# zzzzxxxx111/Rover-SLAM

Measured on AMD Instinct MI355X. Metric: frames/s SuperPoint+LightGlue 640x480, higher is better.
Workload: dtype f32; 1 GPU; configs[3] per GPU: 33 synthetic 640x480 u8 frames resident in HBM, SuperPoint extract (Kmax=1024, thr=0.0005) + LightGlue match of 32 consecutive pairs (9 layers, filter 0.1); 32 frames counted per GPU per step; seeded synthetic weights (centred descriptor head + calibrated LightGlue law, frames shifted by multiples of 8 px); the same resident frames every step (compute-bound path, no data-depend; frames_per_gpu=32, kmax=1024, lg_fold_wo=1, pairing=calibrated

## Files before the change

include/rover_fe.h:

```cpp
#ifndef ROVER_FE_H
#define ROVER_FE_H
#include <stddef.h>
#include <stdint.h>

#ifdef __cplusplus
extern "C" {
#endif

typedef struct rfe_ctx rfe_ctx;

typedef enum {
    RFE_OK = 0,
    RFE_ERR_INVALID = -1,
    RFE_ERR_NO_DEVICE = -2,
    RFE_ERR_HIP = -3,
    RFE_ERR_IO = -4,
    RFE_ERR_NO_WEIGHTS = -5,
    RFE_ERR_OOM = -6
} rfe_status;

#define RFE_DESC_DIM 256
#define RFE_KIND_SUPERPOINT 1
#define RFE_KIND_LIGHTGLUE 2

int rfe_init(int device, rfe_ctx** out);
void rfe_destroy(rfe_ctx* ctx);
const char* rfe_last_error(rfe_ctx* ctx);
const char* rfe_version(void);

int rfe_load_weights(rfe_ctx* ctx, const char* sp_path, const char* lg_path);
int rfe_load_onnx(rfe_ctx* ctx, const char* sp_path, const char* lg_path);
int rfe_set_weights(rfe_ctx* ctx, int kind, const float* blob, int64_t count);
int64_t rfe_weight_count(int kind);
uint64_t rfe_weights_id(rfe_ctx* ctx, int kind);

typedef struct rfe_hparams {
    int32_t sp_max_keypoints;
    float sp_detection_threshold;
    int32_t sp_nms_radius;
    int32_t sp_remove_borders;
    int32_t sp_topk_always;
    int32_t lg_layers;
    int32_t lg_heads;
    float lg_filter_threshold;
} rfe_hparams;
int rfe_get_hparams(rfe_ctx* ctx, rfe_hparams* out);
int rfe_set_hparams(rfe_ctx* ctx, const rfe_hparams* in);

#define RFE_OPT_LG_FOLD_WO 1
#define RFE_OPT_LG_FP16X2 2
#define RFE_OPT_HOST_GRAPH 3
int rfe_set_option(rfe_ctx* ctx, int option, int value);
int rfe_get_option(rfe_ctx* ctx, int option, int* value);

int rfe_set_stream(rfe_ctx* ctx, void* hip_stream);
int rfe_synchronize(rfe_ctx* ctx);
int rfe_malloc(rfe_ctx* ctx, size_t bytes, void** dev_ptr);
int rfe_free(rfe_ctx* ctx, void* dev_ptr);
int rfe_host_malloc(size_t bytes, void** host_ptr);
void rfe_host_free(void* host_ptr);
int64_t rfe_workspace_bytes(rfe_ctx* ctx);
int rfe_memcpy_h2d(rfe_ctx* ctx, void* dst_dev, const void* src_host, size_t bytes);
int rfe_memcpy_d2h(rfe_ctx* ctx, void* dst_host, const void* src_dev, size_t bytes);

int rfe_extract_u8(rfe_ctx* ctx, const uint8_t* img, int H, int W, int stride, int B, int Kmax,
                   float thr, int32_t* n, int32_t* kxy, float* score, float* desc);
int rfe_extract_u8_dev(rfe_ctx* ctx, const uint8_t* img_dev, int H, int W, int stride, int B,
                       int Kmax, float thr, int32_t* n_dev, int32_t* kxy_dev, float* score_dev,
                       float* desc_dev);

int rfe_extract_f32(rfe_ctx* ctx, const float* img, int H, int W, int stride, int B, int Kmax,
                    float thr, int32_t* n, int32_t* kxy, float* score, float* desc);
int rfe_extract_f32_dev(rfe_ctx* ctx, const float* img_dev, int H, int W, int stride, int B,
                        int Kmax, float thr, int32_t* n_dev, int32_t* kxy_dev, float* score_dev,
                        float* desc_dev);

int rfe_extract_u8_bin(rfe_ctx* ctx, const uint8_t* img, int H, int W, int stride, int B, int Kmax, float thr, int32_t* n,
                       int32_t* kxy, float* score, float* desc, uint8_t* desc_bin);
int rfe_extract_u8_bin_dev(rfe_ctx* ctx, const uint8_t* img_dev, int H, int W, int stride, int B, int Kmax, float thr,
                           int32_t* n_dev, int32_t* kxy_dev, float* score_dev, float* desc_dev, uint8_t* desc_bin_dev);

#define RFE_MAX_LEVELS 16
int rfe_pyramid_geometry(int H, int W, int nlevels, float scale_factor, int32_t* level_h, int32_t* level_w, float* level_scale);
int rfe_extract_pyramid_u8(rfe_ctx* ctx, const uint8_t* img, int H, int W, int stride, int B, int nlevels, float scale_factor,
                           const int32_t* kmax, float thr, int32_t* n, int32_t* level_n, float* kpts, int32_t* octave,
                           float* score, float* desc, uint8_t* levels);
int rfe_extract_pyramid_u8_dev(rfe_ctx* ctx, const uint8_t* img_dev, int H, int W, int stride, int B, int nlevels, float scale_factor,
                               const int32_t* kmax, float thr, int32_t* n_dev, int32_t* level_n_dev, float* kpts_dev,
                               int32_t* octave_dev, float* score_dev, float* desc_dev, uint8_t* levels_dev);

int rfe_match(rfe_ctx* ctx, const float* k0n, const float* k1n, const float* d0, const float* d1,
              const int32_t* m, const int32_t* n, int P, int Mmax, int Nmax, float filter_thr,
              int32_t* S, int32_t* pairs, float* ms);
int rfe_match_dev(rfe_ctx* ctx, const float* k0n, const float* k1n, const float* d0,
                  const float* d1, const int32_t* m, const int32_t* n, int P, int Mmax, int Nmax,
                  float filter_thr, int32_t* S, int32_t* pairs, float* ms);

int rfe_match_fused(rfe_ctx* ctx, const float* kpts0_xy, int M, const float* kpts1_xy, int N,
                    const float* desc0, const float* desc1, int rows, int cols, float filter_thr,
                    float match_thresh, int32_t* vnMatches12);

int rfe_extract_match_stream_dev(rfe_ctx* ctx, const uint8_t* img_dev, int H, int W, int stride,
                                 int B, int Kmax, float thr, float filter_thr, int32_t* n_dev,
                                 int32_t* kxy_dev, float* score_dev, float* desc_dev,
                                 int32_t* S_dev, int32_t* pairs_dev, float* ms_dev);

int rfe_stereo_match(rfe_ctx* ctx, const uint8_t* imgL, const uint8_t* imgR, int H, int W, int stride,
                     const float* kL, int N, const float* kR, int Nr, const float* dL, const float* dR,
                     float mb, float mbf, float* uRight, float* depth);
int rfe_stereo_match_dev(rfe_ctx* ctx, const uint8_t* imgL, const uint8_t* imgR, int H, int W, int stride,
                         const float* kL, int N, const float* kR, int Nr, const float* dL, const float* dR,
                         float mb, float mbf, float* uRight, float* depth);

int rfe_stereo_frame_dev(rfe_ctx* ctx, const uint8_t* imgL_dev, const uint8_t* imgR_dev, int H, int W, int stride, int Kmax,
                         float thr, float filter_thr, float mb, float mbf, int reset, int32_t* n_dev, int32_t* kxy_dev,
                         float* score_dev, float* desc_dev, float* uRight_dev, float* depth_dev, int32_t* S_dev,
                         int32_t* pairs_dev, float* ms_dev);

#define RFE_STEREO_SAD_LEVEL  0
#define RFE_STEREO_SAD_LEVEL0 1
int rfe_stereo_match_pyramid(rfe_ctx* ctx, const uint8_t* levelsL, const uint8_t* levelsR, int H, int W, int nlevels, float scale_factor,
                             const float* kL, const int32_t* octL, int N, const float* kR, const int32_t* octR, int Nr,
                             const float* dL, const float* dR, float mb, float mbf, int sad_source, float* uRight, float* depth);
int rfe_stereo_match_pyramid_dev(rfe_ctx* ctx, const uint8_t* levelsL, const uint8_t* levelsR, int H, int W, int nlevels, float scale_factor,
                                 const float* kL, const int32_t* octL, int N, const float* kR, const int32_t* octR, int Nr,
                                 const float* dL, const float* dR, float mb, float mbf, int sad_source, float* uRight, float* depth);
int rfe_stereo_frame_pyramid_dev(rfe_ctx* ctx, const uint8_t* imgL_dev, const uint8_t* imgR_dev, int H, int W, int stride,
                                 int nlevels, float scale_factor, const int32_t* kmax, float thr, float filter_thr, float mb, float mbf,
                                 int sad_source, int reset, int32_t* n_dev, int32_t* level_n_dev, float* kpts_dev, int32_t* octave_dev,
                                 float* score_dev, float* desc_dev, float* uRight_dev, float* depth_dev, int32_t* S_dev,
                                 int32_t* pairs_dev, float* ms_dev);

int rfe_l2_distance_matrix(rfe_ctx* ctx, const float* a, int M, const float* b, int N, float* out);
int rfe_binarize_descriptors(rfe_ctx* ctx, const float* desc, int rows, uint8_t* out);

int rfe_search_candidates(rfe_ctx* ctx, const float* q, int Nq, const float* f, int Nf, const int32_t* offsets,
                          const int32_t* cand, const uint8_t* skip, int32_t* best_idx, float* best_dist, float* second_dist);
int rfe_distinctive_descriptors(rfe_ctx* ctx, const float* desc, const int32_t* offsets, int Np, int32_t* best, float* median);

int rfe_l2_distance_matrix_dev(rfe_ctx* ctx, const float* a_dev, int M, const float* b_dev, int N, float* out_dev);
int rfe_binarize_descriptors_dev(rfe_ctx* ctx, const float* desc_dev, int rows, uint8_t* out_dev);
int rfe_search_candidates_dev(rfe_ctx* ctx, const float* q_dev, int Nq, const float* f_dev, int Nf, const int32_t* offsets_dev,
                              const int32_t* cand_dev, const uint8_t* skip_dev, int32_t* best_idx_dev, float* best_dist_dev,
                              float* second_dist_dev);
int rfe_distinctive_descriptors_dev(rfe_ctx* ctx, const float* desc_dev, const int32_t* offsets_dev, int Np, int total, int maxn,
                                    int32_t* best_dev, float* median_dev);

int rfe_search_by_projection_dev(rfe_ctx* ctx, const float* q_dev, const float* proj_dev, const float* radius_dev,
                                 const int32_t* pred_level_dev, const uint8_t* observed_dev, int Nq, const float* f_dev,
                                 const float* kpts_dev, const int32_t* kxy_dev, const int32_t* octave_dev, const uint8_t* skip_dev, int Nf,
                                 const int32_t* nf_dev, float min_x, float min_y, float max_x, float max_y, float th_high, int cand_cap,
                                 int32_t* assign_dev, int32_t* best_idx_dev, float* best_dist_dev, float* second_dist_dev,
                                 int32_t* stats_dev);
int rfe_search_by_projection(rfe_ctx* ctx, const float* q, const float* proj, const float* radius, const int32_t* pred_level,
                             const uint8_t* observed, int Nq, const float* f, const float* kpts, const int32_t* kxy, const int32_t* octave,
                             const uint8_t* skip, int Nf, float min_x, float min_y, float max_x, float max_y, float th_high,
                             int32_t* assign, int32_t* best_idx, float* best_dist, float* second_dist, int32_t* stats);

#define RFE_PROJ_INVZ 0
#define RFE_PROJ_DIV 1
#define RFE_DIST_FLOAT 0
#define RFE_DIST_TRUNC 1
typedef struct rfe_sim3_params {
    float quat[4];
    float t[3];
    float ow[3];
    float fx, fy, cx, cy;
    float min_x, min_y, max_x, max_y;
    int32_t th;
    int32_t nlevels;
    float log_scale_factor;
    float scale_factors[RFE_MAX_LEVELS];
    int32_t proj_mode, dist_mode;
} rfe_sim3_params;
int rfe_search_by_projection_sim3_dev(rfe_ctx* ctx, const rfe_sim3_params* params, const float* q_dev, const float* pw_dev,
                                      const float* normal_dev, const float* min_dist_dev, const float* max_dist_dev,
                                      const float* scale_dist_dev, const uint8_t* valid_dev, int Np, const float* f_dev, const float* kpts_dev, const int32_t* kxy_dev,
                                      const uint8_t* matched_in_dev, int Nf, const int32_t* nf_dev, float th_accept, int cand_cap,
                                      int32_t* matched_dev, int32_t* best_idx_dev, float* best_dist_dev, float* second_dist_dev,
                                      float* proj_dev, float* radius_dev, int32_t* level_dev, int32_t* reject_dev, int32_t* stats_dev);
int rfe_search_by_projection_sim3(rfe_ctx* ctx, const rfe_sim3_params* params, const float* q, const float* pw, const float* normal,
                                  const float* min_dist, const float* max_dist, const float* scale_dist, const uint8_t* valid, int Np,
                                  const float* f,
                                  const float* kpts, const int32_t* kxy, const uint8_t* matched_in, int Nf, float th_accept,
                                  int32_t* matched, int32_t* best_idx, float* best_dist, float* second_dist, float* proj, float* radius,
                                  int32_t* level, int32_t* reject, int32_t* stats);

typedef struct rfe_pool rfe_pool;
#define RFE_POOL_AUTO 0
#define RFE_POOL_RCCL 1
#define RFE_POOL_COPY 2
int rfe_pool_create(const int* devices, int n, rfe_pool** out);
void rfe_pool_destroy(rfe_pool* pool);
const char* rfe_pool_last_error(rfe_pool* pool);
int rfe_pool_size(rfe_pool* pool);
rfe_ctx* rfe_pool_ctx(rfe_pool* pool, int member);
int rfe_pool_has_rccl(rfe_pool* pool);
int rfe_pool_set_weights(rfe_pool* pool, int kind, const float* blob, int64_t count);
int rfe_pool_load_weights(rfe_pool* pool, const char* sp_path, const char* lg_path);
int rfe_pool_set_option(rfe_pool* pool, int option, int value);
int rfe_pool_set_hparams(rfe_pool* pool, const rfe_hparams* in);
int rfe_pool_shard(int F, int n, int member, int* first_frame, int* frames, int* pairs);
int rfe_pool_extract_match_stream(rfe_pool* pool, const uint8_t* img_host, int H, int W, int stride, int F, int Kmax, float thr,
                                  float filter_thr, int transport, int32_t* n, int32_t* kxy, float* score, float* desc,
                                  int32_t* S, int32_t* pairs, float* ms);

int rfe_profile_enable(rfe_ctx* ctx, int on);
int rfe_profile_filter(rfe_ctx* ctx, const char* stage);
int rfe_profile_reset(rfe_ctx* ctx);
int rfe_profile_read(rfe_ctx* ctx, char* names, size_t names_cap, double* ms, int64_t* calls, int cap);

int rfe_k_conv3x3(rfe_ctx* ctx, const float* in_dev, int B, int H, int W, int Cin,
                  const float* w_oihw_host, const float* bias_host, int Cout, int relu, int pool,
                  float* out_dev);
int rfe_k_linear(rfe_ctx* ctx, const float* a_dev, int M, int K, const float* w_nk_host,
                 const float* bias_host, int N, int relu, float* out_dev);
int rfe_k_scoremap(rfe_ctx* ctx, const uint8_t* img_dev, int H, int W, int stride, int B,
                   float* scoremap_dev ,
                   float* nms_dev , float* descmap_dev );
int rfe_k_select(rfe_ctx* ctx, const float* nms_dev , int B, int H, int W, int Kmax, float thr, int topk_always,
                 int32_t* n_dev, int32_t* kxy_dev, float* score_dev);
int rfe_k_select_keys(rfe_ctx* ctx, const float* nms_dev , int B, int H, int W, int Kmax, float thr, int topk_always,
                      int32_t* n_dev, int32_t* kxy_dev, float* score_dev);
int rfe_k_lightglue_taps(rfe_ctx* ctx, const float* k0n, const float* k1n, const float* d0,
                         const float* d1, int M, int N, float* x0_dev, float* x1_dev,
                         float* scores_dev );

int rfe_k_lightglue_ffn(rfe_ctx* ctx, int layer, int cross, const float* x_dev, const float* second_dev, int rows, float* out_dev);
int rfe_k_attention(rfe_ctx* ctx, const float* q_dev, const float* k_dev, const float* v_dev, int ld, float* out_dev, int nseq, int Lq, int Lk,
                    const int32_t* qlen_dev, const int32_t* klen_dev, const int32_t* kv_map_dev, const float* rope_dev);
int rfe_k_lightglue_self_attention(rfe_ctx* ctx, int layer, const float* x_dev, const float* csn_dev, const int32_t* lens_dev, int nseq, int L,
                                   float* qkv_out_dev, float* ctx_out_dev, int32_t* qk_rotated);
int rfe_k_lightglue_assign(rfe_ctx* ctx, const float* sim_dev, const float* x_dev, const float* wm_dev, const float* bm_dev, const int32_t* lens_dev,
                           int P, int L, float thr, int cap, int scores_pair, int32_t sentinel, float* z_dev, float* rowlse_dev, float* collse_dev,
                           float* mx0_dev, int32_t* a0_dev, int32_t* a1_dev, int32_t* S_dev, int32_t* pairs_dev, float* ms_dev, float* scores_dev);
int rfe_k_set_lightglue_tap(rfe_ctx* ctx, int pair, float* x0_dev, float* x1_dev, float* scores_dev);
int rfe_k_pool_inject_gather_failure(rfe_pool* pool, int member);
int rfe_k_onnx_convert(const char* path, int kind, int weights_only, float* blob, rfe_hparams* hp, char* err, int errlen);

#ifdef __cplusplus
}
#endif
#endif
```

rover-slam_amd/capi.py:

```python
import ctypes as C
import os

import numpy as np

_HERE = os.path.dirname(os.path.abspath(__file__))
LIB_PATH = os.environ.get("RFE_LIBRARY") or os.path.join(_HERE, "librover_fe.so")

KIND_SUPERPOINT, KIND_LIGHTGLUE = 1, 2
OPT_LG_FOLD_WO = 1
OPT_LG_FP16X2 = 2
OPT_HOST_GRAPH = 3

EXPORTS = [
    "rfe_init", "rfe_destroy", "rfe_last_error", "rfe_version", "rfe_load_weights", "rfe_load_onnx", "rfe_set_weights",
    "rfe_weight_count", "rfe_weights_id", "rfe_get_hparams", "rfe_set_hparams", "rfe_set_option", "rfe_get_option", "rfe_set_stream", "rfe_synchronize", "rfe_malloc", "rfe_free", "rfe_host_malloc", "rfe_host_free", "rfe_workspace_bytes", "rfe_memcpy_h2d",
    "rfe_memcpy_d2h", "rfe_extract_u8", "rfe_extract_u8_dev", "rfe_extract_f32", "rfe_extract_f32_dev", "rfe_extract_u8_bin", "rfe_extract_u8_bin_dev",
    "rfe_pyramid_geometry", "rfe_extract_pyramid_u8", "rfe_extract_pyramid_u8_dev", "rfe_match", "rfe_match_dev", "rfe_match_fused",
    "rfe_extract_match_stream_dev", "rfe_stereo_match", "rfe_stereo_match_dev", "rfe_stereo_frame_dev", "rfe_stereo_match_pyramid", "rfe_stereo_match_pyramid_dev", "rfe_stereo_frame_pyramid_dev",
    "rfe_l2_distance_matrix", "rfe_binarize_descriptors",
    "rfe_search_candidates", "rfe_distinctive_descriptors",
    "rfe_l2_distance_matrix_dev", "rfe_binarize_descriptors_dev", "rfe_search_candidates_dev", "rfe_distinctive_descriptors_dev",
    "rfe_search_by_projection", "rfe_search_by_projection_dev", "rfe_search_by_projection_sim3", "rfe_search_by_projection_sim3_dev",
    "rfe_pool_create", "rfe_pool_destroy", "rfe_pool_last_error", "rfe_pool_size", "rfe_pool_ctx", "rfe_pool_has_rccl", "rfe_pool_set_weights",
    "rfe_pool_load_weights", "rfe_pool_set_option", "rfe_pool_set_hparams", "rfe_pool_shard", "rfe_pool_extract_match_stream",
    "rfe_profile_enable", "rfe_profile_filter", "rfe_profile_reset", "rfe_profile_read",
    "rfe_k_conv3x3", "rfe_k_linear", "rfe_k_scoremap", "rfe_k_select", "rfe_k_select_keys", "rfe_k_lightglue_taps", "rfe_k_set_lightglue_tap", "rfe_k_lightglue_ffn", "rfe_k_attention", "rfe_k_lightglue_self_attention", "rfe_k_lightglue_assign", "rfe_k_pool_inject_gather_failure", "rfe_k_onnx_convert",
]

if not os.path.exists(LIB_PATH):
    raise ImportError(f"{LIB_PATH} is missing: build it with `python -c 'import __graft_entry__ as g; g.build()'` "
                      "(rover-slam_amd/csrc/Makefile). There is no CPU fallback.")

lib = C.CDLL(LIB_PATH)

_vp, _fp, _ip, _u8p = C.c_void_p, C.c_void_p, C.c_void_p, C.c_void_p
lib.rfe_init.argtypes = [C.c_int, C.POINTER(C.c_void_p)]
lib.rfe_destroy.argtypes = [C.c_void_p]
lib.rfe_destroy.restype = None
lib.rfe_last_error.argtypes = [C.c_void_p]
lib.rfe_last_error.restype = C.c_char_p
lib.rfe_version.restype = C.c_char_p
lib.rfe_load_weights.argtypes = [C.c_void_p, C.c_char_p, C.c_char_p]
lib.rfe_set_weights.argtypes = [C.c_void_p, C.c_int, _fp, C.c_int64]
lib.rfe_weight_count.argtypes = [C.c_int]
lib.rfe_weight_count.restype = C.c_int64
lib.rfe_weights_id.restype = C.c_uint64
lib.rfe_weights_id.argtypes = [C.c_void_p, C.c_int]


class HParams(C.Structure):
    _fields_ = [("sp_max_keypoints", C.c_int32), ("sp_detection_threshold", C.c_float), ("sp_nms_radius", C.c_int32),
                ("sp_remove_borders", C.c_int32), ("sp_topk_always", C.c_int32), ("lg_layers", C.c_int32), ("lg_heads", C.c_int32), ("lg_filter_threshold", C.c_float)]

    def as_dict(self):
        return {k: getattr(self, k) for k, _ in self._fields_}


lib.rfe_get_hparams.argtypes = [C.c_void_p, C.POINTER(HParams)]
lib.rfe_set_hparams.argtypes = [C.c_void_p, C.POINTER(HParams)]
lib.rfe_pool_set_hparams.argtypes = [C.c_void_p, C.POINTER(HParams)]
lib.rfe_set_option.argtypes = [C.c_void_p, C.c_int, C.c_int]
lib.rfe_get_option.argtypes = [C.c_void_p, C.c_int, C.POINTER(C.c_int)]
lib.rfe_set_stream.argtypes = [C.c_void_p, C.c_void_p]
lib.rfe_synchronize.argtypes = [C.c_void_p]
lib.rfe_malloc.argtypes = [C.c_void_p, C.c_size_t, C.POINTER(C.c_void_p)]
lib.rfe_free.argtypes = [C.c_void_p, C.c_void_p]
lib.rfe_memcpy_h2d.argtypes = [C.c_void_p, C.c_void_p, C.c_void_p, C.c_size_t]
lib.rfe_memcpy_d2h.argtypes = [C.c_void_p, C.c_void_p, C.c_void_p, C.c_size_t]
_ext = [C.c_void_p, _u8p, C.c_int, C.c_int, C.c_int, C.c_int, C.c_int, C.c_float, _ip, _ip, _fp, _fp]
lib.rfe_extract_u8.argtypes = _ext
lib.rfe_extract_f32.argtypes = _ext
lib.rfe_extract_f32_dev.argtypes = _ext
lib.rfe_extract_u8_dev.argtypes = _ext
lib.rfe_extract_u8_bin.argtypes = _ext + [_u8p]
lib.rfe_extract_u8_bin_dev.argtypes = _ext + [_u8p]
lib.rfe_pyramid_geometry.argtypes = [C.c_int, C.c_int, C.c_int, C.c_float, _ip, _ip, _fp]
_pyr = [C.c_void_p, _u8p, C.c_int, C.c_int, C.c_int, C.c_int, C.c_int, C.c_float, _ip, C.c_float, _ip, _ip, _fp, _ip, _fp, _fp, _u8p]
lib.rfe_extract_pyramid_u8.argtypes = _pyr
lib.rfe_extract_pyramid_u8_dev.argtypes = _pyr
_mt = [C.c_void_p, _fp, _fp, _fp, _fp, _ip, _ip, C.c_int, C.c_int, C.c_int, C.c_float, _ip, _ip, _fp]
lib.rfe_match.argtypes = _mt
lib.rfe_match_dev.argtypes = _mt
lib.rfe_match_fused.argtypes = [C.c_void_p, _fp, C.c_int, _fp, C.c_int, _fp, _fp, C.c_int, C.c_int, C.c_float,
                                C.c_float, _ip]
lib.rfe_extract_match_stream_dev.argtypes = [C.c_void_p, _u8p, C.c_int, C.c_int, C.c_int, C.c_int, C.c_int, C.c_float,
                                             C.c_float, _ip, _ip, _fp, _fp, _ip, _ip, _fp]
_st = [C.c_void_p, _u8p, _u8p, C.c_int, C.c_int, C.c_int, _fp, C.c_int, _fp, C.c_int, _fp, _fp, C.c_float, C.c_float, _fp, _fp]
lib.rfe_stereo_match.argtypes = _st
lib.rfe_stereo_match_dev.argtypes = _st
lib.rfe_stereo_frame_dev.argtypes = [C.c_void_p, _u8p, _u8p, C.c_int, C.c_int, C.c_int, C.c_int, C.c_float, C.c_float, C.c_float, C.c_float,
                                     C.c_int, _ip, _ip, _fp, _fp, _fp, _fp, _ip, _ip, _fp]
_stp = [C.c_void_p, _u8p, _u8p, C.c_int, C.c_int, C.c_int, C.c_float, _fp, _ip, C.c_int, _fp, _ip, C.c_int, _fp, _fp, C.c_float, C.c_float,
        C.c_int, _fp, _fp]
lib.rfe_stereo_match_pyramid.argtypes = _stp
lib.rfe_stereo_match_pyramid_dev.argtypes = _stp
lib.rfe_stereo_frame_pyramid_dev.argtypes = [C.c_void_p, _u8p, _u8p, C.c_int, C.c_int, C.c_int, C.c_int, C.c_float, _ip, C.c_float, C.c_float,
                                             C.c_float, C.c_float, C.c_int, C.c_int, _ip, _ip, _fp, _ip, _fp, _fp, _fp, _fp, _ip, _ip, _fp]
lib.rfe_l2_distance_matrix.argtypes = [C.c_void_p, _fp, C.c_int, _fp, C.c_int, _fp]
lib.rfe_binarize_descriptors.argtypes = [C.c_void_p, _fp, C.c_int, _u8p]
lib.rfe_search_candidates.argtypes = [C.c_void_p, _fp, C.c_int, _fp, C.c_int, _ip, _ip, _u8p, _ip, _fp, _fp]
lib.rfe_distinctive_descriptors.argtypes = [C.c_void_p, _fp, _ip, C.c_int, _ip, _fp]
lib.rfe_l2_distance_matrix_dev.argtypes = [C.c_void_p, _fp, C.c_int, _fp, C.c_int, _fp]
lib.rfe_binarize_descriptors_dev.argtypes = [C.c_void_p, _fp, C.c_int, _u8p]
lib.rfe_search_candidates_dev.argtypes = [C.c_void_p, _fp, C.c_int, _fp, C.c_int, _ip, _ip, _u8p, _ip, _fp, _fp]
lib.rfe_distinctive_descriptors_dev.argtypes = [C.c_void_p, _fp, _ip, C.c_int, C.c_int, C.c_int, _ip, _fp]
_psq = [C.c_void_p, _fp, _fp, _fp, _ip, _u8p, C.c_int, _fp, _fp, _ip, _ip, _u8p, C.c_int]
_psb = [C.c_float, C.c_float, C.c_float, C.c_float, C.c_float]
lib.rfe_search_by_projection.argtypes = _psq + _psb + [_ip, _ip, _fp, _fp, _ip]
lib.rfe_search_by_projection_dev.argtypes = _psq + [_ip] + _psb + [C.c_int, _ip, _ip, _fp, _fp, _ip]


MAX_LEVELS = 16
PROJ_INVZ, PROJ_DIV = 0, 1
DIST_FLOAT, DIST_TRUNC = 0, 1


class Sim3Params(C.Structure):
    _fields_ = [("quat", C.c_float * 4), ("t", C.c_float * 3), ("ow", C.c_float * 3), ("fx", C.c_float), ("fy", C.c_float), ("cx", C.c_float),
                ("cy", C.c_float), ("min_x", C.c_float), ("min_y", C.c_float), ("max_x", C.c_float), ("max_y", C.c_float), ("th", C.c_int32),
                ("nlevels", C.c_int32), ("log_scale_factor", C.c_float), ("scale_factors", C.c_float * MAX_LEVELS),
                ("proj_mode", C.c_int32), ("dist_mode", C.c_int32)]


def sim3_params(quat, t, ow, intrinsics, bounds, th, scale_factors=(1.0,), log_scale_factor=0.0, proj_mode=PROJ_INVZ, dist_mode=DIST_FLOAT,
                nlevels=None):
    p = Sim3Params()
    p.quat[:] = [float(v) for v in quat]; p.t[:] = [float(v) for v in t]; p.ow[:] = [float(v) for v in ow]
    p.fx, p.fy, p.cx, p.cy = (float(v) for v in intrinsics)
    p.min_x, p.min_y, p.max_x, p.max_y = (float(v) for v in bounds)
    p.th, p.nlevels, p.log_scale_factor = int(th), len(scale_factors) if nlevels is None else int(nlevels), float(log_scale_factor)
    for l, v in enumerate(list(scale_factors)[:MAX_LEVELS]):
        p.scale_factors[l] = float(v)
    p.proj_mode, p.dist_mode = int(proj_mode), int(dist_mode)
    return p


_s3q = [C.c_void_p, C.POINTER(Sim3Params), _fp, _fp, _fp, _fp, _fp, _fp, _u8p, C.c_int, _fp, _fp, _ip, _u8p, C.c_int]
_s3o = [_ip, _ip, _fp, _fp, _fp, _fp, _ip, _ip, _ip]
lib.rfe_search_by_projection_sim3.argtypes = _s3q + [C.c_float] + _s3o
lib.rfe_search_by_projection_sim3_dev.argtypes = _s3q + [_ip, C.c_float, C.c_int] + _s3o
lib.rfe_profile_enable.argtypes = [C.c_void_p, C.c_int]
lib.rfe_profile_filter.argtypes = [C.c_void_p, C.c_char_p]
lib.rfe_profile_reset.argtypes = [C.c_void_p]
lib.rfe_profile_read.argtypes = [C.c_void_p, C.c_char_p, C.c_size_t, C.POINTER(C.c_double), C.POINTER(C.c_int64), C.c_int]
lib.rfe_k_conv3x3.argtypes = [C.c_void_p, _fp, C.c_int, C.c_int, C.c_int, C.c_int, _fp, _fp, C.c_int, C.c_int, C.c_int, _fp]
lib.rfe_k_linear.argtypes = [C.c_void_p, _fp, C.c_int, C.c_int, _fp, _fp, C.c_int, C.c_int, _fp]
lib.rfe_k_scoremap.argtypes = [C.c_void_p, _u8p, C.c_int, C.c_int, C.c_int, C.c_int, _fp, _fp, _fp]
lib.rfe_k_select.argtypes = [C.c_void_p, _fp, C.c_int, C.c_int, C.c_int, C.c_int, C.c_float, C.c_int, _ip, _ip, _fp]
lib.rfe_k_select_keys.argtypes = lib.rfe_k_select.argtypes
lib.rfe_k_lightglue_taps.argtypes = [C.c_void_p, _fp, _fp, _fp, _fp, C.c_int, C.c_int, _fp, _fp, _fp]
lib.rfe_k_set_lightglue_tap.argtypes = [C.c_void_p, C.c_int, _fp, _fp, _fp]
lib.rfe_k_lightglue_ffn.argtypes = [C.c_void_p, C.c_int, C.c_int, _fp, _fp, C.c_int, _fp]
lib.rfe_k_lightglue_self_attention.argtypes = [C.c_void_p, C.c_int, _fp, _fp, C.c_void_p, C.c_int, C.c_int, _fp, _fp, C.POINTER(C.c_int32)]
lib.rfe_k_lightglue_assign.argtypes = [C.c_void_p, _fp, _fp, _fp, _fp, _ip, C.c_int, C.c_int, C.c_float, C.c_int, C.c_int, C.c_int32,
                                       _fp, _fp, _fp, _fp, _ip, _ip, _ip, _ip, _fp, _fp]
lib.rfe_k_attention.argtypes = [C.c_void_p, _fp, _fp, _fp, C.c_int, _fp, C.c_int, C.c_int, C.c_int, C.c_void_p, C.c_void_p, C.c_void_p, _fp]


POOL_AUTO, POOL_RCCL, POOL_COPY = 0, 1, 2
lib.rfe_pool_create.argtypes = [C.POINTER(C.c_int), C.c_int, C.POINTER(C.c_void_p)]
lib.rfe_pool_destroy.argtypes = [C.c_void_p]
lib.rfe_pool_destroy.restype = None
lib.rfe_pool_last_error.argtypes = [C.c_void_p]
lib.rfe_pool_last_error.restype = C.c_char_p
lib.rfe_pool_size.argtypes = [C.c_void_p]
lib.rfe_pool_ctx.argtypes = [C.c_void_p, C.c_int]
lib.rfe_pool_ctx.restype = C.c_void_p
lib.rfe_pool_has_rccl.argtypes = [C.c_void_p]
lib.rfe_k_pool_inject_gather_failure.argtypes = [C.c_void_p, C.c_int]
lib.rfe_load_onnx.argtypes = [C.c_void_p, C.c_char_p, C.c_char_p]
lib.rfe_k_onnx_convert.argtypes = [C.c_char_p, C.c_int, C.c_int, C.POINTER(C.c_float), C.c_void_p, C.c_char_p, C.c_int]
lib.rfe_host_malloc.argtypes = [C.c_size_t, C.POINTER(C.c_void_p)]
lib.rfe_host_free.argtypes = [C.c_void_p]
lib.rfe_host_free.restype = None
lib.rfe_workspace_bytes.argtypes = [C.c_void_p]
lib.rfe_workspace_bytes.restype = C.c_int64
lib.rfe_pool_set_weights.argtypes = [C.c_void_p, C.c_int, _fp, C.c_int64]
lib.rfe_pool_load_weights.argtypes = [C.c_void_p, C.c_char_p, C.c_char_p]
lib.rfe_pool_set_option.argtypes = [C.c_void_p, C.c_int, C.c_int]
lib.rfe_pool_shard.argtypes = [C.c_int, C.c_int, C.c_int, C.POINTER(C.c_int), C.POINTER(C.c_int), C.POINTER(C.c_int)]
lib.rfe_pool_extract_match_stream.argtypes = [C.c_void_p, _u8p, C.c_int, C.c_int, C.c_int, C.c_int, C.c_int, C.c_float, C.c_float, C.c_int,
                                              _ip, _ip, _fp, _fp, _ip, _ip, _fp]


class RfeError(RuntimeError):
    pass


def _addr(a):
    if a is None:
        return None
    if isinstance(a, int):
        return a
    if isinstance(a, np.ndarray):
        assert a.flags["C_CONTIGUOUS"]
        return a.ctypes.data
    if hasattr(a, "data_ptr"):
        return a.data_ptr()
    raise TypeError(type(a))


class DevBuf:

    def __init__(self, ctx, nbytes):
        self.ctx, self.nbytes = ctx, int(nbytes)
        p = C.c_void_p()
        ctx._chk(lib.rfe_malloc(ctx.h, self.nbytes, C.byref(p)))
        self.ptr = p.value

    def upload(self, arr):
        arr = np.ascontiguousarray(arr)
        assert arr.nbytes <= self.nbytes
        self.ctx._chk(lib.rfe_memcpy_h2d(self.ctx.h, self.ptr, arr.ctypes.data, arr.nbytes))
        return self

    def download(self, shape, dtype):
        out = np.empty(shape, dtype)
        assert out.nbytes <= self.nbytes
        self.ctx._chk(lib.rfe_memcpy_d2h(self.ctx.h, out.ctypes.data, self.ptr, out.nbytes))
        return out

    def free(self):
        if self.ptr:
            lib.rfe_free(self.ctx.h, self.ptr)
            self.ptr = None


def split_levels(flat, level_h, level_w):
    out, off = [], 0
    for h, w in zip(level_h, level_w):
        out.append(flat[:, off:off + int(h) * int(w)].reshape(flat.shape[0], int(h), int(w)))
        off += int(h) * int(w)
    return out


class StereoStream:

    def __init__(self, ctx, H, W, kmax=1024, mb=0.11, mbf=0.11 * 435.0, thr=0.0005, filter_thr=0.1):
        self.ctx, self.H, self.W, self.K = ctx, H, W, kmax
        self.mb, self.mbf, self.thr, self.filter_thr = mb, mbf, thr, filter_thr
        K = kmax
        self._spec = [("n", np.int32, (2,)), ("kxy", np.int32, (2, K, 2)), ("score", np.float32, (2, K)), ("desc", np.float32, (2, K, 256)),
                      ("u_right", np.float32, (K,)), ("depth", np.float32, (K,)), ("S", np.int32, (1,)), ("pairs", np.int32, (K, 2)),
                      ("ms", np.float32, (K,))]
        self.bufs = {name: ctx.alloc(int(np.prod(shape)) * np.dtype(dt).itemsize) for name, dt, shape in self._spec}
        self.first = True

    def push(self, img_l_dev, img_r_dev, stride=None, reset=False):
        b = self.bufs
        self.ctx._chk(lib.rfe_stereo_frame_dev(self.ctx.h, _addr(img_l_dev), _addr(img_r_dev), self.H, self.W, stride or self.W, self.K,
                                               self.thr, self.filter_thr, self.mb, self.mbf, int(reset or self.first), b["n"].ptr,
                                               b["kxy"].ptr, b["score"].ptr, b["desc"].ptr, b["u_right"].ptr, b["depth"].ptr,
                                               b["S"].ptr, b["pairs"].ptr, b["ms"].ptr))
        self.first = False

    def results(self):
        self.ctx.synchronize()
        out = {name: self.bufs[name].download(shape, dt) for name, dt, shape in self._spec}
        out["S"] = int(out["S"][0])
        return out

    def close(self):
        for b in self.bufs.values():
            b.free()
        self.bufs = {}


STEREO_SAD_LEVEL, STEREO_SAD_LEVEL0 = 0, 1


class StereoPyramidStream:

    def __init__(self, ctx, H, W, nlevels=8, scale_factor=1.2, kmax=128, mb=0.11, mbf=0.11 * 435.0, thr=0.0005, filter_thr=0.1,
                 sad_source=STEREO_SAD_LEVEL):
        self.ctx, self.H, self.W, self.L, self.sf = ctx, H, W, int(nlevels), scale_factor
        self.kmax = np.full((max(self.L, 1),), int(kmax), np.int32) if np.isscalar(kmax) else np.ascontiguousarray(kmax, np.int32)
        self.mb, self.mbf, self.thr, self.filter_thr, self.sad_source = mb, mbf, thr, filter_thr, sad_source
        K = self.K = int(self.kmax.sum())
        self._spec = [("n", np.int32, (2,)), ("level_n", np.int32, (2, max(self.L, 1))), ("kpts", np.float32, (2, K, 2)),
                      ("octave", np.int32, (2, K)), ("score", np.float32, (2, K)), ("desc", np.float32, (2, K, 256)),
                      ("u_right", np.float32, (K,)), ("depth", np.float32, (K,)), ("S", np.int32, (1,)), ("pairs", np.int32, (K, 2)),
                      ("ms", np.float32, (K,))]
        self.bufs = {name: ctx.alloc(max(int(np.prod(shape)), 1) * np.dtype(dt).itemsize) for name, dt, shape in self._spec}
        self.first = True

    def push(self, img_l_dev, img_r_dev, stride=None, reset=False):
        b = self.bufs
        self.ctx._chk(lib.rfe_stereo_frame_pyramid_dev(self.ctx.h, _addr(img_l_dev), _addr(img_r_dev), self.H, self.W, stride or self.W, self.L,
                                                       self.sf, self.kmax.ctypes.data, self.thr, self.filter_thr, self.mb, self.mbf,
                                                       self.sad_source, int(reset or self.first), b["n"].ptr, b["level_n"].ptr, b["kpts"].ptr,
                                                       b["octave"].ptr, b["score"].ptr, b["desc"].ptr, b["u_right"].ptr, b["depth"].ptr,
                                                       b["S"].ptr, b["pairs"].ptr, b["ms"].ptr))
        self.first = False

    def results(self):
        self.ctx.synchronize()
        out = {name: self.bufs[name].download(shape, dt) for name, dt, shape in self._spec}
        out["S"] = int(out["S"][0])
        return out

    def close(self):
        for b in self.bufs.values():
            b.free()
        self.bufs = {}


MAX_LEVELS = 16


def pyramid_geometry(H, W, nlevels, scale_factor):
    L = max(int(nlevels), 1)
    h, w, s = np.zeros((L,), np.int32), np.zeros((L,), np.int32), np.zeros((L,), np.float32)
    rc = lib.rfe_pyramid_geometry(H, W, nlevels, scale_factor, h.ctypes.data, w.ctypes.data, s.ctypes.data)
    if rc < 0:
        raise RfeError(f"rfe_pyramid_geometry({H}, {W}, {nlevels}, {scale_factor}) failed ({rc})")
    return h, w, s


def pool_shard(F, n, member):
    a, b, c = C.c_int(), C.c_int(), C.c_int()
    rc = lib.rfe_pool_shard(F, n, member, C.byref(a), C.byref(b), C.byref(c))
    if rc < 0:
        raise RfeError(f"rfe_pool_shard({F}, {n}, {member}) failed ({rc})")
    return a.value, b.value, c.value


class Pool:

    def __init__(self, devices):
        devs = (C.c_int * len(devices))(*devices)
        h = C.c_void_p()
        rc = lib.rfe_pool_create(devs, len(devices), C.byref(h))
        if rc != 0:
            raise RfeError(f"rfe_pool_create failed ({rc}): {lib.rfe_pool_last_error(None).decode()}")
        self.h = h

    def close(self):
        if self.h:
            lib.rfe_pool_destroy(self.h)
            self.h = None

    def __del__(self):
        try:
            self.close()
        except Exception:
            pass

    def _chk(self, rc):
        if rc < 0:
            raise RfeError(f"librover_fe pool error {rc}: {lib.rfe_pool_last_error(self.h).decode()}")
        return rc

    @property
    def size(self):
        return lib.rfe_pool_size(self.h)

    @property
    def has_rccl(self):
        return bool(lib.rfe_pool_has_rccl(self.h))

    def set_weights(self, kind, blob):
        blob = np.ascontiguousarray(blob, np.float32)
        self._chk(lib.rfe_pool_set_weights(self.h, kind, blob.ctypes.data, blob.size))

    def set_option(self, option, value):
        self._chk(lib.rfe_pool_set_option(self.h, option, int(value)))

    def set_hparams(self, **kw):
        h = HParams()
        rc = lib.rfe_get_hparams(lib.rfe_pool_ctx(self.h, 0), C.byref(h))
        if rc < 0:
            raise RfeError(f"rfe_get_hparams on pool member 0 failed ({rc})")
        for k, v in kw.items():
            if not hasattr(h, k):
                raise KeyError(k)
            setattr(h, k, v)
        self._chk(lib.rfe_pool_set_hparams(self.h, C.byref(h)))

    def extract_match_stream(self, frames_u8, kmax=1024, thr=0.0005, filter_thr=0.1, transport=POOL_AUTO, with_desc=True):
        img = np.ascontiguousarray(frames_u8, np.uint8)
        F, H, W = img.shape
        P = max(F - 1, 1)
        out = {"n": np.zeros((F,), np.int32), "kxy": np.zeros((F, kmax, 2), np.int32), "S": np.zeros((P,), np.int32),
               "pairs": np.zeros((P, kmax, 2), np.int32), "ms": np.zeros((P, kmax), np.float32)}
        if with_desc:
            out["score"] = np.zeros((F, kmax), np.float32)
            out["desc"] = np.zeros((F, kmax, 256), np.float32)
        self._chk(lib.rfe_pool_extract_match_stream(self.h, img.ctypes.data, H, W, W, F, kmax, thr, filter_thr, transport, out["n"].ctypes.data,
                                                    out["kxy"].ctypes.data, out["score"].ctypes.data if with_desc else None,
                                                    out["desc"].ctypes.data if with_desc else None, out["S"].ctypes.data,
                                                    out["pairs"].ctypes.data, out["ms"].ctypes.data))
        return out


class Context:

    def __init__(self, device=0):
        h = C.c_void_p()
        rc = lib.rfe_init(device, C.byref(h))
        if rc != 0:
            raise RfeError(f"rfe_init failed ({rc}): {lib.rfe_last_error(None).decode()}")
        self.h = h

    def close(self):
        if self.h:
            lib.rfe_destroy(self.h)
            self.h = None

    def __del__(self):
        try:
            self.close()
        except Exception:
            pass

    def _chk(self, rc):
        if rc < 0:
            raise RfeError(f"librover_fe error {rc}: {lib.rfe_last_error(self.h).decode()}")
        return rc

    def set_weights(self, kind, blob):
        blob = np.ascontiguousarray(blob, np.float32)
        self._chk(lib.rfe_set_weights(self.h, kind, blob.ctypes.data, blob.size))

    def load_weights(self, sp_path=None, lg_path=None):
        self._chk(lib.rfe_load_weights(self.h, sp_path.encode() if sp_path else None, lg_path.encode() if lg_path else None))

    def get_hparams(self):
        h = HParams()
        self._chk(lib.rfe_get_hparams(self.h, C.byref(h)))
        return h.as_dict()

    def set_hparams(self, **kw):
        h = HParams()
        self._chk(lib.rfe_get_hparams(self.h, C.byref(h)))
        for k, v in kw.items():
            if not hasattr(h, k):
                raise KeyError(k)
            setattr(h, k, v)
        self._chk(lib.rfe_set_hparams(self.h, C.byref(h)))

    def set_option(self, option, value):
        self._chk(lib.rfe_set_option(self.h, option, int(value)))

    def get_option(self, option):
        v = C.c_int()
        self._chk(lib.rfe_get_option(self.h, option, C.byref(v)))
        return v.value

    def set_stream(self, stream_ptr):
        self._chk(lib.rfe_set_stream(self.h, stream_ptr))
# ... 220 lines not shown
```

rover-slam_amd/csrc/api_extract.hip:

```cpp
#include <string.h>
#include "api_internal.h"

using namespace rfe;

namespace rfe {

static void sp_layout(Bump& a, int B, int H, int W, SpBuffers& b) {
    const size_t hw = (size_t)B * H * W, cells = hw / 64;
    b.p1 = a.take<float>(hw / 4 * 64); b.a2 = a.take<float>(hw / 4 * 64);
    b.p2 = a.take<float>(hw / 16 * 64); b.a3 = a.take<float>(hw / 16 * 128);
    b.p3 = a.take<float>(cells * 128); b.a4 = a.take<float>(cells * 128); b.f4 = a.take<float>(cells * 128);
    b.pa = a.take<float>(cells * 256); b.da = a.take<float>(cells * 256); b.dmap = a.take<float>(cells * 256);
    b.logits = a.take<float>(cells * 65);
    b.smap = a.take<float>(hw); b.nmap = a.take<float>(hw); b.ss = a.take<float>(hw);
    b.mask = a.take<uint8_t>(hw); b.supp = a.take<uint8_t>(hw);
    b.cand_score = a.take<float>(hw); b.cand_idx = a.take<int32_t>(hw);
    b.sel_keys = a.take<unsigned long long>((size_t)B * 4096); b.sel_n = a.take<int32_t>(B);
}
size_t sp_ws_bytes(int B, int H, int W) { SpBuffers b; return layout_bytes([&](Bump& a) { sp_layout(a, B, H, W, b); }); }
int sp_carve(rfe_ctx* c, int B, int H, int W, SpBuffers& b) {
    return ws_carve(c, &c->ws_sp, &c->ws_sp_bytes, [&](Bump& a) { sp_layout(a, B, H, W, b); });
}

GemmArgs gemm_plain(const float* A, int lda, const float* Bw, int ldb, const float* bias, float* C, int ldc, int M, int N, int K) {
    GemmArgs g;
    memset(&g, 0, sizeof(g));
    g.A = A; g.lda = lda; g.B = Bw; g.ldb = ldb; g.bias = bias; g.C = C; g.ldc = ldc;
    g.M = M; g.N = N; g.K = K; g.alpha = 1.0f; g.batch = 1;
    return g;
}

int sp_check(rfe_ctx* c, int H, int W, int B, int Kmax) {
    if (!c) return RFE_ERR_INVALID;
    if (!c->has_sp) return fail(c, RFE_ERR_NO_WEIGHTS, "SuperPoint weights not loaded (rfe_load_weights / rfe_set_weights)");
    if (H < 8 || W < 8 || B <= 0) return fail(c, RFE_ERR_INVALID, "extract: H and W must be at least 8, B > 0");
    if (Kmax <= 0 || Kmax > 4096) return fail(c, RFE_ERR_INVALID, "extract: Kmax must be in 1..4096");
    return RFE_OK;
}

int sp_forward_maps(rfe_ctx* c, const void* img, int H, int W, int stride, int B, SpBuffers& b, bool join, bool& forked, bool img_f32, long long frame_step,
                    float thr, bool want_maps) {
    forked = false;
    int rc = sp_carve(c, B, H, W, b);
    if (rc) return rc;
    hipStream_t s = c->stream;
    const SpWeightsDev& w = c->sp;
    const int H1 = H / 2, W1 = W / 2, H2 = H1 / 2, W2 = W1 / 2, Hc = H2 / 2, Wc = W2 / 2, cells = B * Hc * Wc;
    { ProfScope p(c, "conv1ab");
      launch_conv1ab_fused(s, img, img_f32, stride, B, H, W, w.conv1a_w, w.bias[L_1A], w.packed[L_1B], w.bias[L_1B], b.p1, frame_step); }
    { ProfScope p(c, "conv2a"); launch_conv3x3(s, b.p1, B, H1, W1, 64, w.packed[L_2A], w.bias[L_2A], 64, true, kSpLayers[L_2A].pool, b.a2, L_2A); }
    { ProfScope p(c, "conv2b"); launch_conv3x3(s, b.a2, B, H1, W1, 64, w.packed[L_2B], w.bias[L_2B], 64, true, kSpLayers[L_2B].pool, b.p2, L_2B); }
    { ProfScope p(c, "conv3a"); launch_conv3x3(s, b.p2, B, H2, W2, 64, w.packed[L_3A], w.bias[L_3A], 128, true, kSpLayers[L_3A].pool, b.a3, L_3A); }
    { ProfScope p(c, "conv3b"); launch_conv3x3(s, b.a3, B, H2, W2, 128, w.packed[L_3B], w.bias[L_3B], 128, true, kSpLayers[L_3B].pool, b.p3, L_3B); }
    { ProfScope p(c, "conv4a"); launch_conv3x3(s, b.p3, B, Hc, Wc, 128, w.packed[L_4A], w.bias[L_4A], 128, true, kSpLayers[L_4A].pool, b.a4, L_4A); }
    { ProfScope p(c, "conv4b"); launch_conv3x3(s, b.a4, B, Hc, Wc, 128, w.packed[L_4B], w.bias[L_4B], 128, true, kSpLayers[L_4B].pool, b.f4, L_4B); }
    const bool fork = !(c->prof && c->prof_filter.empty());
    hipStream_t sd = fork ? c->side_stream : s;
    if (fork) { RFE_HIP(c, hipEventRecord(c->ev_fork, s)); RFE_HIP(c, hipStreamWaitEvent(sd, c->ev_fork, 0)); }
    { ProfScope p(c, "convDa", sd); launch_conv3x3(sd, b.f4, B, Hc, Wc, 128, w.packed[L_DA], w.bias[L_DA], 256, true, kSpLayers[L_DA].pool, b.da, L_DA); }
    { ProfScope p(c, "convDb", sd); launch_gemm_nt(sd, gemm_plain(b.da, 256, w.packed[L_DB], 256, w.bias[L_DB], b.dmap, 256, cells, 256, 256)); }
    { ProfScope p(c, "sp_post", sd); launch_descmap_norm(sd, b.dmap, cells); }
    if (fork) RFE_HIP(c, hipEventRecord(c->ev_join, sd));
    { ProfScope p(c, "convPa"); launch_conv3x3(s, b.f4, B, Hc, Wc, 128, w.packed[L_PA], w.bias[L_PA], 256, true, kSpLayers[L_PA].pool, b.pa, L_PA); }
    { ProfScope p(c, "convPb"); launch_gemm_nt(s, gemm_plain(b.pa, 256, w.packed[L_PB], 256, w.bias[L_PB], b.logits, 65, cells, 65, 256)); }
    { ProfScope p(c, "sp_post");
      if (B <= 4 && c->hp.sp_nms_radius == 4) {
          if (!c->sp_cnt) { RFE_HIP(c, hipMalloc((void**)&c->sp_cnt, 8 * sizeof(int32_t))); c->sp_cnt_dirty = true; }
          if (c->sp_cnt_dirty) { RFE_HIP(c, hipMemsetAsync(c->sp_cnt, 0, 8 * sizeof(int32_t), s)); c->sp_cnt_dirty = false; }
          b.tail_fused = launch_sp_tail_lat(s, b.logits, B, Hc, Wc, c->hp.sp_nms_radius, c->hp.sp_remove_borders, thr, (unsigned long long*)b.cand_score, c->sp_cnt,
                                            want_maps ? b.smap : nullptr, want_maps ? b.nmap : nullptr);
          if (b.tail_fused) c->sp_cnt_dirty = true;
      }
      if (!b.tail_fused) {
          launch_softmax65_d2s(s, b.logits, 65, B, Hc, Wc, b.smap);
          launch_nms(s, b.smap, B, 8 * Hc, 8 * Wc, c->hp.sp_nms_radius, c->hp.sp_remove_borders, b.ss, b.mask, b.supp, b.nmap);
      } }
    if (fork && join) RFE_HIP(c, hipStreamWaitEvent(s, c->ev_join, 0));
    forked = fork && !join;
    RFE_HIP(c, hipGetLastError());
    return RFE_OK;
}

int sp_forward(rfe_ctx* c, const void* img, int H, int W, int stride, int B, int Kmax, float thr,
               int32_t* n, int32_t* kxy, float* score, float* desc, uint8_t* desc_bin, bool img_f32, long long frame_step) {
    SpBuffers b;
    bool forked;
    int rc = sp_forward_maps(c, img, H, W, stride, B, b, false, forked, img_f32, frame_step, thr);
    if (rc) return rc;
    const int Hc = H / 2 / 2 / 2, Wc = W / 2 / 2 / 2, Hs = 8 * Hc, Ws = 8 * Wc;
    { ProfScope p(c, "sp_select");
      if (b.tail_fused) {
          launch_select_keys(c->stream, (const unsigned long long*)b.cand_score, c->sp_cnt, B, Hs, Ws, Kmax, c->hp.sp_topk_always != 0, n, kxy, score);
          c->sp_cnt_dirty = false;
      } else
      launch_select(c->stream, b.nmap, B, Hs, Ws, Kmax, thr, b.cand_score, b.cand_idx, n, kxy, score, (int32_t*)b.ss , c->hp.sp_topk_always != 0, b.sel_keys, b.sel_n);
      if (forked) RFE_HIP(c, hipStreamWaitEvent(c->stream, c->ev_join, 0));
      launch_desc_sample(c->stream, b.dmap, B, Hc, Wc, Hs, Ws, n, kxy, Kmax, desc, desc_bin); }
    RFE_HIP(c, hipGetLastError());
    return RFE_OK;
}

}

static int extract_check(rfe_ctx* c, const void* img, int H, int W, int stride, int B, int Kmax, const void* n, const void* kxy, const void* score,
                         const void* desc) {
    int rc = sp_check(c, H, W, B, Kmax);
    if (rc) return rc;
    if (!img || !n || !kxy || !score || !desc || stride < W) return fail(c, RFE_ERR_INVALID, "extract: null pointer or stride < W");
    RFE_HIP(c, hipSetDevice(c->device));
    return RFE_OK;
}

extern "C" int rfe_extract_u8_bin_dev(rfe_ctx* c, const uint8_t* img, int H, int W, int stride, int B, int Kmax,
                                      float thr, int32_t* n, int32_t* kxy, float* score, float* desc, uint8_t* desc_bin) {
    int rc = extract_check(c, img, H, W, stride, B, Kmax, n, kxy, score, desc);
    if (rc) return rc;
    return sp_forward(c, img, H, W, stride, B, Kmax, thr, n, kxy, score, desc, desc_bin);
}

extern "C" int rfe_extract_u8_dev(rfe_ctx* c, const uint8_t* img, int H, int W, int stride, int B, int Kmax,
                                  float thr, int32_t* n, int32_t* kxy, float* score, float* desc) {
    return rfe_extract_u8_bin_dev(c, img, H, W, stride, B, Kmax, thr, n, kxy, score, desc, nullptr);
}

extern "C" int rfe_extract_f32_dev(rfe_ctx* c, const float* img, int H, int W, int stride, int B, int Kmax,
                                   float thr, int32_t* n, int32_t* kxy, float* score, float* desc) {
    int rc = extract_check(c, img, H, W, stride, B, Kmax, n, kxy, score, desc);
    if (rc) return rc;
    return sp_forward(c, img, H, W, stride, B, Kmax, thr, n, kxy, score, desc, nullptr, true);
}

static int extract_host(rfe_ctx* c, const void* img, size_t px, int H, int W, int stride, int B, int Kmax, float thr, int32_t* n, int32_t* kxy,
                        float* score, float* desc, uint8_t* desc_bin) {
    int rc = extract_check(c, img, H, W, stride, B, Kmax, n, kxy, score, desc);
    if (rc) return rc;
    const size_t K = (size_t)B * Kmax;
    uint8_t *d_img, *d_b; int32_t *d_n, *d_k; float *d_s, *d_d;
    HostIo io(c, HostIo::PINNED);
    io.image(d_img, (const uint8_t*)img, (size_t)W * px, (size_t)B * H, (size_t)stride * px);
    io.out(d_n, n, B); io.out(d_k, kxy, K * 2); io.out(d_s, score, K);
    io.out(d_d, desc, K * 256, true);
    io.out_opt(d_b, desc_bin, K * 256);
    if ((rc = io.upload())) return rc;
    if ((rc = ensure_ws(c, &c->ws_sp, &c->ws_sp_bytes, sp_ws_bytes(B, H, W)))) return rc;
    int thr_bits; memcpy(&thr_bits, &thr, 4);
    const std::string key = px == 1 ? host_graph_key(c, "xu8", {H, W, B, Kmax, thr_bits, desc_bin != nullptr}) : host_graph_key(c, "xf32", {H, W, B, Kmax, thr_bits});
    if ((rc = run_host_graph(c, c->g_extract, key, [&] { return sp_forward(c, d_img, H, W, W, B, Kmax, thr, d_n, d_k, d_s, d_d, d_b, px == 4); }))) return rc;
    return io.download();
}

extern "C" int rfe_extract_u8(rfe_ctx* c, const uint8_t* img, int H, int W, int stride, int B, int Kmax, float thr,
                              int32_t* n, int32_t* kxy, float* score, float* desc) {
    return extract_host(c, img, 1, H, W, stride, B, Kmax, thr, n, kxy, score, desc, nullptr);
}
extern "C" int rfe_extract_u8_bin(rfe_ctx* c, const uint8_t* img, int H, int W, int stride, int B, int Kmax, float thr,
                                  int32_t* n, int32_t* kxy, float* score, float* desc, uint8_t* desc_bin) {
    return extract_host(c, img, 1, H, W, stride, B, Kmax, thr, n, kxy, score, desc, desc_bin);
}
extern "C" int rfe_extract_f32(rfe_ctx* c, const float* img, int H, int W, int stride, int B, int Kmax, float thr,
                               int32_t* n, int32_t* kxy, float* score, float* desc) {
    return extract_host(c, img, 4, H, W, stride, B, Kmax, thr, n, kxy, score, desc, nullptr);
}

extern "C" int rfe_pyramid_geometry(int H, int W, int nlevels, float scale_factor, int32_t* level_h, int32_t* level_w, float* level_scale) {
    return pyramid_geometry(H, W, nlevels, scale_factor, level_h, level_w, level_scale);
}

namespace rfe {

int pyr_check(rfe_ctx* c, int H, int W, int stride, int B, int L, float sf, const int32_t* kmax, PyrPlan& P) {
    if (!c) return RFE_ERR_INVALID;
    if (!c->has_sp) return fail(c, RFE_ERR_NO_WEIGHTS, "SuperPoint weights not loaded (rfe_load_weights / rfe_set_weights)");
    if (L < 1 || L > RFE_MAX_LEVELS) return fail(c, RFE_ERR_INVALID, "extract_pyramid: nlevels must be in 1..16");
    if (L > 1 && !(sf > 1.0f && sf <= 4.0f)) return fail(c, RFE_ERR_INVALID, "extract_pyramid: scale_factor must be in (1, 4] when nlevels > 1");
    if (H < 8 || W < 8 || B < 1 || stride < W) return fail(c, RFE_ERR_INVALID, "extract_pyramid: H and W must be at least 8, B > 0, stride >= W");
    if (!kmax) return fail(c, RFE_ERR_INVALID, "extract_pyramid: null pointer");
    P.L = L; P.Ktot = 0;
    for (int l = 0; l < L; ++l) {
        if (kmax[l] < 0 || kmax[l] > 4096) return fail(c, RFE_ERR_INVALID, "extract_pyramid: every kmax[l] must be in 0..4096");
        P.kmax[l] = kmax[l]; P.Ktot += kmax[l];
    }
    if (P.Ktot == 0) return fail(c, RFE_ERR_INVALID, "extract_pyramid: every kmax[l] is 0");
    if (pyramid_geometry(H, W, L, sf, P.h, P.w, P.s) != RFE_OK) return fail(c, RFE_ERR_INVALID, "extract_pyramid: a level rounds to zero pixels");
    P.frame = 0;
    for (int l = 0; l < L; ++l) {
        P.off[l] = P.frame; P.frame += (size_t)P.h[l] * P.w[l];
        P.run[l] = P.kmax[l] > 0 && P.h[l] >= 8 && P.w[l] >= 8;
    }
    return RFE_OK;
}

struct PyrStage { uint8_t* levels; int32_t *n[RFE_MAX_LEVELS], *kxy[RFE_MAX_LEVELS]; float *sc[RFE_MAX_LEVELS], *desc[RFE_MAX_LEVELS]; };
static void pyr_layout(Bump& a, const PyrPlan& P, int B, bool own_levels, PyrStage& st) {
    st.levels = own_levels ? a.take<uint8_t>((size_t)B * P.frame) : nullptr;
    for (int l = 0; l < P.L; ++l) {
        if (!P.run[l]) continue;
        st.n[l] = a.take<int32_t>((size_t)B); st.kxy[l] = a.take<int32_t>((size_t)B * P.kmax[l] * 2);
        st.sc[l] = a.take<float>((size_t)B * P.kmax[l]); st.desc[l] = a.take<float>((size_t)B * P.kmax[l] * 256);
    }
}

int pyr_prepare(rfe_ctx* c, int H, int W, int B, float sf, const PyrPlan& P, bool own_levels) {
    int rc;
    if ((rc = ensure_ws(c, &c->ws_sp, &c->ws_sp_bytes, sp_ws_bytes(B, H, W)))) return rc;
    PyrStage st;
    if ((rc = ensure_ws(c, &c->ws_pyr, &c->ws_pyr_bytes, layout_bytes([&](Bump& a) { pyr_layout(a, P, B, own_levels, st); })))) return rc;
    if (!c->sp_cnt) { RFE_HIP(c, hipMalloc((void**)&c->sp_cnt, 8 * sizeof(int32_t))); c->sp_cnt_dirty = true; }
    int sf_bits; memcpy(&sf_bits, &sf, 4);
    const std::string key = std::to_string(H) + "x" + std::to_string(W) + "|" + std::to_string(P.L) + "|" + std::to_string(P.L > 1 ? sf_bits : 0);
    if (P.L > 1 && key != c->ptab_key) {
        std::vector<int2> tab;
        pyramid_tables(P.L, P.h, P.w, tab, c->ptab_off);
        c->ptab_key.clear();
        const void* before = c->ws_ptab;
        if ((rc = ensure_ws(c, &c->ws_ptab, &c->ws_ptab_bytes, tab.size() * sizeof(int2)))) return rc;
        if (before == c->ws_ptab) RFE_HIP(c, hipStreamSynchronize(c->stream));
        RFE_HIP(c, hipMemcpy(c->ws_ptab, tab.data(), tab.size() * sizeof(int2), hipMemcpyHostToDevice));
        c->ptab_key = key;
    }
    return RFE_OK;
}

int pyr_forward(rfe_ctx* c, const uint8_t* img, int H, int W, int stride, int B, const PyrPlan& P, float thr, uint8_t* lv, bool copy_level0,
                int32_t* n, int32_t* level_n, float* kpts, int32_t* octave, float* score, float* desc, long long img_frame) {
    if (img_frame == 0) img_frame = (long long)stride * H;
    hipStream_t s = c->stream;
    const bool side = !(c->prof && c->prof_filter.empty());
    hipStream_t sc = side ? c->side_stream : s;
    if (side) { RFE_HIP(c, hipEventRecord(c->ev_fork, s)); RFE_HIP(c, hipStreamWaitEvent(sc, c->ev_fork, 0)); }
    { ProfScope p(c, "sp_pyramid", sc);
      if (copy_level0) launch_pyr_resample(sc, img, img_frame, stride, H, W, lv, (long long)P.frame, H, W, B, nullptr, nullptr);
      const int2* tab = (const int2*)c->ws_ptab;
      for (int l = 1; l < P.L; ++l) {
          const uint8_t* src = l == 1 ? img : lv + P.off[l - 1];
          const long long src_frame = l == 1 ? img_frame : (long long)P.frame;
          const int src_stride = l == 1 ? stride : P.w[l - 1];
          launch_pyr_resample(sc, src, src_frame, src_stride, P.h[l - 1], P.w[l - 1], lv + P.off[l], (long long)P.frame, P.h[l], P.w[l], B,
                              tab + c->ptab_off[l], tab + c->ptab_off[l] + P.w[l]);
      } }
    if (side) RFE_HIP(c, hipEventRecord(c->ev_pyr, sc));
    PyrMergeArgs m;
    memset(&m, 0, sizeof(m));
    m.L = P.L; m.Ktot = P.Ktot;
    PyrStage st;
    Bump a(c->ws_pyr);
    pyr_layout(a, P, B, lv == (uint8_t*)c->ws_pyr, st);
    int rc;
    bool joined = !side;
    for (int l = 0; l < P.L; ++l) {
        m.kmax[l] = P.kmax[l]; m.scale[l] = P.s[l];
        if (!P.run[l]) continue;
        int32_t* ln = st.n[l]; int32_t* lk = st.kxy[l]; float* ls = st.sc[l]; float* ld = st.desc[l];
        if (l >= 1 && !joined) { RFE_HIP(c, hipStreamWaitEvent(s, c->ev_pyr, 0)); joined = true; }
        if (l == 0) rc = sp_forward(c, img, H, W, stride, B, P.kmax[0], thr, ln, lk, ls, ld, nullptr, false, img_frame);
        else rc = sp_forward(c, lv + P.off[l], P.h[l], P.w[l], P.w[l], B, P.kmax[l], thr, ln, lk, ls, ld, nullptr, false, (long long)P.frame);
        if (rc) return rc;
        m.n[l] = ln; m.kxy[l] = lk; m.sc[l] = ls; m.desc_l[l] = ld;
    }
    if (!joined) RFE_HIP(c, hipStreamWaitEvent(s, c->ev_pyr, 0));
    m.n_out = n; m.level_n = level_n; m.kpts = kpts; m.octave = octave; m.score = score; m.desc = desc;
    { ProfScope p(c, "sp_merge"); launch_pyr_merge(s, m, B); }
    RFE_HIP(c, hipGetLastError());
    return RFE_OK;
}

}

static int pyr_entry_check(rfe_ctx* c, const void* img, int H, int W, int stride, int B, int nlevels, float scale_factor, const int32_t* kmax, const void* n,
                           const void* kpts, const void* octave, const void* score, const void* desc, PyrPlan& P) {
    int rc = pyr_check(c, H, W, stride, B, nlevels, scale_factor, kmax, P);
    if (rc) return rc;
    if (!img || !n || !kpts || !octave || !score || !desc) return fail(c, RFE_ERR_INVALID, "extract_pyramid: null pointer");
    RFE_HIP(c, hipSetDevice(c->device));
    return RFE_OK;
}

extern "C" int rfe_extract_pyramid_u8_dev(rfe_ctx* c, const uint8_t* img, int H, int W, int stride, int B, int nlevels, float scale_factor,
                                          const int32_t* kmax, float thr, int32_t* n, int32_t* level_n, float* kpts, int32_t* octave,
                                          float* score, float* desc, uint8_t* levels) {
    PyrPlan P;
    int rc = pyr_entry_check(c, img, H, W, stride, B, nlevels, scale_factor, kmax, n, kpts, octave, score, desc, P);
    if (rc) return rc;
    if ((rc = pyr_prepare(c, H, W, B, scale_factor, P, levels == nullptr))) return rc;
    return pyr_forward(c, img, H, W, stride, B, P, thr, levels ? levels : (uint8_t*)c->ws_pyr, levels != nullptr, n, level_n, kpts, octave,
                       score, desc);
}

extern "C" int rfe_extract_pyramid_u8(rfe_ctx* c, const uint8_t* img, int H, int W, int stride, int B, int nlevels, float scale_factor,
                                      const int32_t* kmax, float thr, int32_t* n, int32_t* level_n, float* kpts, int32_t* octave,
                                      float* score, float* desc, uint8_t* levels) {
    PyrPlan P;
    int rc = pyr_entry_check(c, img, H, W, stride, B, nlevels, scale_factor, kmax, n, kpts, octave, score, desc, P);
    if (rc) return rc;
    const size_t K = (size_t)B * P.Ktot;
    uint8_t *d_img, *d_v; int32_t *d_n, *d_ln, *d_o; float *d_k, *d_s, *d_d;
    HostIo io(c, HostIo::PINNED);
    io.image(d_img, img, (size_t)W, (size_t)B * H, (size_t)stride);
    io.out(d_n, n, B); io.out(d_ln, level_n, (size_t)B * nlevels); io.out(d_k, kpts, K * 2); io.out(d_o, octave, K); io.out(d_s, score, K);
    io.out(d_d, desc, K * 256, true);
    io.out_opt(d_v, levels, (size_t)B * P.frame);
    if ((rc = pyr_prepare(c, H, W, B, scale_factor, P, levels == nullptr))) return rc;
    if ((rc = io.upload())) return rc;
    if ((rc = pyr_forward(c, d_img, H, W, W, B, P, thr, d_v ? d_v : (uint8_t*)c->ws_pyr, d_v != nullptr, d_n, d_ln, d_k, d_o, d_s, d_d))) return rc;
    return io.download();
}
```

rover-slam_amd/csrc/api_hooks.hip:

```cpp
#include <algorithm>
#include "api_internal.h"

using namespace rfe;

extern "C" int rfe_k_conv3x3(rfe_ctx* c, const float* in, int B, int H, int W, int Cin, const float* w, const float* bias,
                             int Cout, int relu, int pool, float* out) {
    if (!c) return RFE_ERR_INVALID;
    if ((Cin != 16 && Cin != 32 && Cin != 64 && Cin != 128) || (Cout % 64)) return fail(c, RFE_ERR_INVALID, "k_conv3x3: Cin in {16,32,64,128}, Cout % 64 == 0");
    RFE_HIP(c, hipSetDevice(c->device));
    std::vector<float> packed;
    pack_conv3x3_weights(w, Cin, Cout, pool != 0, packed);
    float *dw, *db;
    int rc = ws_carve(c, &c->ws_tmp, &c->ws_tmp_bytes, [&](Bump& a) { dw = a.take<float>(packed.size()); db = a.take<float>(Cout); });
    if (rc) return rc;
    RFE_HIP(c, hipMemcpyAsync(dw, packed.data(), packed.size() * 4, hipMemcpyHostToDevice, c->stream));
    RFE_HIP(c, hipMemcpyAsync(db, bias, (size_t)Cout * 4, hipMemcpyHostToDevice, c->stream));
    launch_conv3x3(c->stream, in, B, H, W, Cin, dw, db, Cout, relu != 0, pool != 0, out, 0);
    RFE_HIP(c, hipGetLastError());
    RFE_HIP(c, hipStreamSynchronize(c->stream));
    return RFE_OK;
}

extern "C" int rfe_k_linear(rfe_ctx* c, const float* a, int M, int K, const float* w, const float* bias, int N, int relu,
                            float* out) {
    if (!c) return RFE_ERR_INVALID;
    if (K % 32) return fail(c, RFE_ERR_INVALID, "k_linear: K % 32 == 0 required");
    RFE_HIP(c, hipSetDevice(c->device));
    float *dw, *db;
    int rc = ws_carve(c, &c->ws_tmp, &c->ws_tmp_bytes, [&](Bump& a) { dw = a.take<float>((size_t)N * K); db = a.take<float>(N); });
    if (rc) return rc;
    RFE_HIP(c, hipMemcpyAsync(dw, w, (size_t)N * K * 4, hipMemcpyHostToDevice, c->stream));
    if (bias) RFE_HIP(c, hipMemcpyAsync(db, bias, (size_t)N * 4, hipMemcpyHostToDevice, c->stream));
    GemmArgs g = gemm_plain(a, K, dw, K, bias ? db : nullptr, out, N, M, N, K);
    g.relu = relu;
    launch_gemm_nt(c->stream, g);
    RFE_HIP(c, hipGetLastError());
    RFE_HIP(c, hipStreamSynchronize(c->stream));
    return RFE_OK;
}

extern "C" int rfe_k_scoremap(rfe_ctx* c, const uint8_t* img, int H, int W, int stride, int B, float* scoremap,
                              float* nms, float* descmap) {
    int rc = sp_check(c, H, W, B, 1);
    if (rc) return rc;
    RFE_HIP(c, hipSetDevice(c->device));
    SpBuffers b;
    bool forked;
    if ((rc = sp_forward_maps(c, img, H, W, stride, B, b, true, forked, false, 0, 0.0005f, true))) return rc;
    const size_t hw = (size_t)B * (H / 8 * 8) * (W / 8 * 8);
    if (scoremap) RFE_HIP(c, hipMemcpyAsync(scoremap, b.smap, hw * 4, hipMemcpyDeviceToDevice, c->stream));
    if (nms) RFE_HIP(c, hipMemcpyAsync(nms, b.nmap, hw * 4, hipMemcpyDeviceToDevice, c->stream));
    if (descmap) RFE_HIP(c, hipMemcpyAsync(descmap, b.dmap, hw / 64 * 256 * 4, hipMemcpyDeviceToDevice, c->stream));
    RFE_HIP(c, hipStreamSynchronize(c->stream));
    return RFE_OK;
}

extern "C" int rfe_k_select(rfe_ctx* c, const float* nms, int B, int H, int W, int Kmax, float thr, int topk_always, int32_t* n, int32_t* kxy,
                            float* score) {
    int rc = sp_check(c, H, W, B, Kmax);
    if (rc) return rc;
    if (!nms || !n || !kxy || !score) return fail(c, RFE_ERR_INVALID, "k_select: null pointer");
    RFE_HIP(c, hipSetDevice(c->device));
    SpBuffers b;
    if ((rc = sp_carve(c, B, H, W, b))) return rc;
    launch_select(c->stream, nms, B, H, W, Kmax, thr, b.cand_score, b.cand_idx, n, kxy, score, (int32_t*)b.ss, topk_always != 0, b.sel_keys, b.sel_n);
    RFE_HIP(c, hipGetLastError());
    RFE_HIP(c, hipStreamSynchronize(c->stream));
    return RFE_OK;
}

extern "C" int rfe_k_select_keys(rfe_ctx* c, const float* nms, int B, int H, int W, int Kmax, float thr, int topk_always, int32_t* n, int32_t* kxy,
                                 float* score) {
    int rc = sp_check(c, H, W, B, Kmax);
    if (rc) return rc;
    if (!nms || !n || !kxy || !score || B > 4) return fail(c, RFE_ERR_INVALID, "k_select_keys: null pointer or more than four frames");
    RFE_HIP(c, hipSetDevice(c->device));
    SpBuffers b;
    if ((rc = sp_carve(c, B, H, W, b))) return rc;
    if (!c->sp_cnt) RFE_HIP(c, hipMalloc((void**)&c->sp_cnt, 8 * sizeof(int32_t)));
    RFE_HIP(c, hipMemsetAsync(c->sp_cnt, 0, 8 * sizeof(int32_t), c->stream));
    launch_keys_from_map(c->stream, nms, B, H * W, thr, (unsigned long long*)b.cand_score, c->sp_cnt);
    launch_select_keys(c->stream, (const unsigned long long*)b.cand_score, c->sp_cnt, B, H, W, Kmax, topk_always != 0, n, kxy, score);
    c->sp_cnt_dirty = false;
    RFE_HIP(c, hipGetLastError());
    RFE_HIP(c, hipStreamSynchronize(c->stream));
    int32_t left[8];
    RFE_HIP(c, hipMemcpy(left, c->sp_cnt, sizeof(left), hipMemcpyDeviceToHost));
    for (int q = 0; q < 8; ++q) if (left[q] != 0) return fail(c, RFE_ERR_HIP, "k_select_keys: the ranking kernel did not leave the candidate counters at zero");
    return RFE_OK;
}

extern "C" int rfe_k_lightglue_ffn(rfe_ctx* c, int layer, int cross, const float* x, const float* second, int rows, float* out) {
    int rc = lg_check(c, 1, 4, 4);
    if (rc) return rc;
    if (layer < 0 || layer >= LG_LAYERS || rows <= 0 || !x || !second || !out) return fail(c, RFE_ERR_INVALID, "k_lightglue_ffn: bad argument");
    RFE_HIP(c, hipSetDevice(c->device));
    const int L = 1024, P = (rows + 2 * L - 1) / (2 * L);
    LgBuffers b;
    if ((rc = lg_carve(c, P, L, b))) return rc;
    const LgLayerDev& Lw = c->lg.L[layer];
    RFE_HIP(c, hipMemcpyAsync(out, x, (size_t)rows * 1024, hipMemcpyDeviceToDevice, c->stream));
    if (cross) lg_ffn(c, b, out, second, rows, Lw.cw1, Lw.cb1, Lw.clng, Lw.clnb, Lw.cw2, Lw.cb2);
    else lg_ffn(c, b, out, second, rows, Lw.w1, Lw.b1, Lw.lng, Lw.lnb, Lw.w2, Lw.b2);
    RFE_HIP(c, hipGetLastError());
    RFE_HIP(c, hipStreamSynchronize(c->stream));
    return RFE_OK;
}

extern "C" int rfe_k_attention(rfe_ctx* c, const float* q, const float* k, const float* v, int ld, float* out, int nseq, int Lq, int Lk,
                               const int32_t* qlen, const int32_t* klen, const int32_t* kv_map, const float* rope) {
    if (!c) return RFE_ERR_INVALID;
    if (!q || !k || !v || !out || nseq <= 0 || Lq <= 0 || Lk <= 0 || ld < 256) return fail(c, RFE_ERR_INVALID, "k_attention: bad argument");
    RFE_HIP(c, hipSetDevice(c->device));
    float* part = nullptr;
    const size_t pb = lg_attention_part_bytes(nseq, Lq);
    if (pb) RFE_HIP(c, hipMalloc((void**)&part, pb));
    launch_lg_attention(c->stream, q, k, v, ld, out, nseq, Lq, Lk, qlen, klen, kv_map, part, rope, c->opt_lg_fp16x2);
    hipError_t e = hipGetLastError();
    if (e == hipSuccess) e = hipStreamSynchronize(c->stream);
    if (part) (void)hipFree(part);
    RFE_HIP(c, e);
    return RFE_OK;
}

extern "C" int rfe_k_set_lightglue_tap(rfe_ctx* c, int pair, float* x0, float* x1, float* scores) {
    if (!c) return RFE_ERR_INVALID;
    if (pair < 0) { c->tap.armed = false; return RFE_OK; }
    c->tap.armed = true; c->tap.pair = pair; c->tap.x0 = x0; c->tap.x1 = x1; c->tap.scores = scores;
    return RFE_OK;
}

extern "C" int rfe_k_lightglue_self_attention(rfe_ctx* c, int layer, const float* x, const float* csn, const int32_t* lens, int nseq, int L,
                                              float* qkv_out, float* ctx_out, int32_t* qk_rotated) {
    int rc = lg_check(c, 1, 4, 4);
    if (rc) return rc;
    if (layer < 0 || layer >= LG_LAYERS || nseq <= 0 || L <= 0 || (L % 4) || !x || !csn || !lens) return fail(c, RFE_ERR_INVALID, "k_lightglue_self_attention: bad argument");
    RFE_HIP(c, hipSetDevice(c->device));
    const int P = (nseq + 1) / 2;
    LgBuffers b;
    if ((rc = lg_carve(c, P, L, b))) return rc;
    const bool rot = lg_self_qkv_attention(c, b, c->lg.L[layer], x, csn, lens, nseq, L);
    RFE_HIP(c, hipGetLastError());
    if (qkv_out) RFE_HIP(c, hipMemcpyAsync(qkv_out, b.qkv, (size_t)nseq * L * 768 * 4, hipMemcpyDeviceToDevice, c->stream));
    if (ctx_out) RFE_HIP(c, hipMemcpyAsync(ctx_out, b.ctx, (size_t)nseq * L * 256 * 4, hipMemcpyDeviceToDevice, c->stream));
    RFE_HIP(c, hipStreamSynchronize(c->stream));
    if (qk_rotated) *qk_rotated = rot ? 1 : 0;
    return RFE_OK;
}

extern "C" int rfe_k_lightglue_assign(rfe_ctx* c, const float* sim, const float* x, const float* wm, const float* bm, const int32_t* lens, int P, int L,
                                      float thr, int cap, int scores_pair, int32_t sentinel, float* z, float* rowlse, float* collse, float* mx0,
                                      int32_t* a0, int32_t* a1, int32_t* S, int32_t* pairs, float* ms, float* scores) {
    if (!c) return RFE_ERR_INVALID;
    if (!sim || !x || !wm || !bm || !lens || P <= 0 || L < 4 || L > 4096 || (L % 4) || cap <= 0 || scores_pair >= P)
        return fail(c, RFE_ERR_INVALID, "k_lightglue_assign: null input, P <= 0, L not a multiple of 4 in [4, 4096], cap <= 0 or scores_pair >= P");
    RFE_HIP(c, hipSetDevice(c->device));
    {
        std::vector<int32_t> hl((size_t)2 * P);
        RFE_HIP(c, hipMemcpy(hl.data(), lens, hl.size() * 4, hipMemcpyDeviceToHost));
        for (int32_t v : hl) if (v < 0 || v > L) return fail(c, RFE_ERR_INVALID, "k_lightglue_assign: a length outside [0, L]");
    }
    const size_t PL = (size_t)P * L, n_scores = scores ? (scores_pair < 0 ? PL * L : (size_t)L * L) : 0;
    LgBuffers b;
    float *dsc = nullptr, *dms; int32_t *dS, *dp;
    int rc = lg_carve(c, P, L, b, [&](Bump& a) {
        dS = a.take<int32_t>(P); dp = a.take<int32_t>((size_t)P * cap * 2); dms = a.take<float>((size_t)P * cap);
        if (n_scores) dsc = a.take<float>(n_scores);
    });
    if (rc) return rc;
    hipStream_t s = c->stream;
    RFE_HIP(c, hipMemcpyAsync(b.sim, sim, PL * L * 4, hipMemcpyDeviceToDevice, s));
    RFE_HIP(c, hipMemcpyAsync(b.x, x, 2 * PL * 1024, hipMemcpyDeviceToDevice, s));
    RFE_HIP(c, hipMemcpyAsync(b.lens, lens, (size_t)2 * P * 4, hipMemcpyDeviceToDevice, s));
    const struct { void* p; size_t words; } fill[] = {{b.z, 2 * PL}, {b.rowlse, PL}, {b.collse, PL}, {b.mx0, PL}, {b.a0, PL}, {b.a1, PL},
                                                      {dS, (size_t)P}, {dp, (size_t)P * cap * 2}, {dms, (size_t)P * cap}, {dsc, n_scores}};
    for (const auto& f : fill)
        if (f.words) RFE_HIP(c, hipMemsetD32Async((hipDeviceptr_t)f.p, sentinel, f.words, s));
    lg_assign_stage(s, b, P, L, thr, cap, dS, dp, dms, dsc, scores_pair, wm, bm);
    RFE_HIP(c, hipGetLastError());
    const struct { void* dst; const void* src; size_t words; } out[] = {{z, b.z, 2 * PL}, {rowlse, b.rowlse, PL}, {collse, b.collse, PL}, {mx0, b.mx0, PL},
                                                                       {a0, b.a0, PL}, {a1, b.a1, PL}, {S, dS, (size_t)P}, {pairs, dp, (size_t)P * cap * 2},
                                                                       {ms, dms, (size_t)P * cap}, {scores, dsc, n_scores}};
    for (const auto& o : out)
        if (o.dst && o.words) RFE_HIP(c, hipMemcpyAsync(o.dst, o.src, o.words * 4, hipMemcpyDeviceToDevice, s));
    RFE_HIP(c, hipStreamSynchronize(s));
    return RFE_OK;
}

extern "C" int rfe_k_lightglue_taps(rfe_ctx* c, const float* k0n, const float* k1n, const float* d0, const float* d1,
                                    int M, int N, float* x0, float* x1, float* scores) {
    int rc = lg_check(c, 1, M, N);
    if (rc) return rc;
    RFE_HIP(c, hipSetDevice(c->device));
    const int L = ((std::max(M, N) + 3) / 4) * 4, cap = std::min(M, N);
    LgBuffers b;
    float *sc, *dms; int32_t *dm, *dn, *dS, *dp;
    if ((rc = lg_carve(c, 1, L, b, [&](Bump& a) {
             sc = a.take<float>((size_t)L * L);
             dm = a.take<int32_t>(1); dn = a.take<int32_t>(1); dS = a.take<int32_t>(1);
             dp = a.take<int32_t>((size_t)cap * 2); dms = a.take<float>(cap);
         }))) return rc;
    RFE_HIP(c, hipMemcpyAsync(dm, &M, 4, hipMemcpyHostToDevice, c->stream));
    RFE_HIP(c, hipMemcpyAsync(dn, &N, 4, hipMemcpyHostToDevice, c->stream));
    RFE_HIP(c, hipStreamSynchronize(c->stream));
    if ((rc = lg_stage(c, b, k0n, k1n, d0, d1, dm, dn, 1, M, N, L))) return rc;
    if ((rc = lg_forward(c, b, 1, L, 0.1f, cap, dS, dp, dms, scores ? sc : nullptr, false, true))) return rc;
    if (x0) RFE_HIP(c, hipMemcpyAsync(x0, b.x, (size_t)M * 1024, hipMemcpyDeviceToDevice, c->stream));
    if (x1) RFE_HIP(c, hipMemcpyAsync(x1, b.x + (size_t)L * 256, (size_t)N * 1024, hipMemcpyDeviceToDevice, c->stream));
    if (scores) RFE_HIP(c, hipMemcpy2DAsync(scores, (size_t)N * 4, sc, (size_t)L * 4, (size_t)N * 4, M, hipMemcpyDeviceToDevice, c->stream));
    RFE_HIP(c, hipStreamSynchronize(c->stream));
    return RFE_OK;
}
```

rover-slam_amd/csrc/api_internal.h:

```cpp
#pragma once
#include <string.h>
#include <algorithm>
#include <initializer_list>
#include "rfe_internal.h"

namespace rfe {

inline size_t al(size_t bytes) { return (bytes + 255) & ~(size_t)255; }

struct Bump {
    char* base; size_t off = 0;
    explicit Bump(void* b) : base((char*)b) {}
    template <typename T> T* take(size_t n) { T* p = base ? (T*)(base + off) : nullptr; off += al(n * sizeof(T)); return p; }
};
template <typename F> size_t layout_bytes(F&& layout) { Bump m(nullptr); layout(m); return m.off; }
template <typename F> int ws_carve(rfe_ctx* c, void** ws, size_t* cur, F&& layout) {
    const int rc = ensure_ws(c, ws, cur, layout_bytes(layout));
    if (rc) return rc;
    Bump a(*ws);
    layout(a);
    return RFE_OK;
}

int ensure_pin(rfe_ctx* c, size_t need);
bool is_lib_pinned(const void* p, size_t bytes);

struct HostIo {
    enum Transport { PINNED, DIRECT };
    HostIo(rfe_ctx* ctx, Transport transport) : c(ctx), t(transport) {}
    template <typename T> void in(T*& dev, const T* host, size_t n) { add(ins, n_in, (void**)&dev, host, n * sizeof(T), true); }
    template <typename T> void in_opt(T*& dev, const T* host, size_t n) { add(ins, n_in, (void**)&dev, host, n * sizeof(T), host != nullptr); }
    template <typename T> void image(T*& dev, const T* host, size_t row_bytes, size_t rows, size_t pitch) {
        add(ins, n_in, (void**)&dev, host, row_bytes * rows, true);
        ins[n_in - 1].row_bytes = row_bytes; ins[n_in - 1].pitch = pitch;
    }
    void cut() { ins[n_in - 1].cut = true; }
    template <typename T> void out(T*& dev, T* host, size_t n, bool to_caller = false) {
        add(outs, n_out, (void**)&dev, host, n * sizeof(T), true);
        outs[n_out - 1].to_caller = to_caller && t == PINNED && is_lib_pinned(host, n * sizeof(T));
    }
    template <typename T> void out_opt(T*& dev, T* host, size_t n) { add(outs, n_out, (void**)&dev, host, n * sizeof(T), host != nullptr); }
    template <typename T> void scratch(T*& dev, size_t n) { add(outs, n_out, (void**)&dev, nullptr, n * sizeof(T), true); }
    int upload();
    int download();

private:
    struct Item { void** dev; void* host; char* p; size_t bytes, row_bytes, pitch; bool carve, cut, to_caller; };
    static constexpr int MAX_ITEMS = 12;
    void add(Item* v, int& n, void** dev, const void* host, size_t bytes, bool carve) {
        if (n >= MAX_ITEMS) abort();
        v[n++] = Item{dev, const_cast<void*>(host), nullptr, bytes, 0, 0, carve, false, false};
    }
    void layout(Bump& a);
    static size_t run_bytes(const Item* first, const Item* last) { return first == last ? first->bytes : (size_t)(last->p - first->p) + al(last->bytes); }
    rfe_ctx* c; Transport t;
    Item ins[MAX_ITEMS], outs[MAX_ITEMS]; int n_in = 0, n_out = 0;
};

constexpr int HOST_GRAPH_REPEATS = 3;
template <typename F>
int run_host_graph(rfe_ctx* c, rfe_ctx::HostGraph& g, const std::string& key, F&& enqueue) {
    if (!c->opt_host_graph || c->prof || c->tap.armed) return enqueue();
    ++g.tick;
    for (auto& sl : g.slot)
        if (sl.exec && sl.key == key) { sl.used = g.tick; RFE_HIP(c, hipGraphLaunch(sl.exec, c->stream)); return RFE_OK; }
    rfe_ctx::HostGraph::Seen* sn = nullptr;
    for (auto& q : g.seen) if (q.count > 0 && q.key == key) sn = &q;
    if (!sn) {
        sn = &g.seen[0];
        for (auto& q : g.seen) if (q.used < sn->used) sn = &q;
        sn->key = key; sn->count = 0;
    }
    sn->used = g.tick;
    if (++sn->count < HOST_GRAPH_REPEATS) return enqueue();
    if (hipStreamBeginCapture(c->stream, hipStreamCaptureModeThreadLocal) != hipSuccess) { (void)hipGetLastError(); sn->count = 0; return enqueue(); }
    const int rc = enqueue();
    hipGraph_t graph = nullptr;
    const hipError_t e = hipStreamEndCapture(c->stream, &graph);
    if (rc != RFE_OK || e != hipSuccess || !graph) {
        if (graph) (void)hipGraphDestroy(graph);
        (void)hipGetLastError();
        sn->count = 0;
        return rc != RFE_OK ? rc : enqueue();
    }
    hipGraphExec_t exec = nullptr;
    const hipError_t ei = hipGraphInstantiate(&exec, graph, nullptr, nullptr, 0);
    (void)hipGraphDestroy(graph);
    if (ei != hipSuccess || !exec) { (void)hipGetLastError(); sn->count = 0; return enqueue(); }
    rfe_ctx::HostGraph::Slot* sl = &g.slot[0];
    for (auto& q : g.slot) { if (!q.exec) { sl = &q; break; } if (q.used < sl->used) sl = &q; }
    if (sl->exec) (void)hipGraphExecDestroy(sl->exec);
    sl->exec = exec; sl->key = key; sl->used = g.tick;
    sn->count = 0; sn->key.clear();
    RFE_HIP(c, hipGraphLaunch(sl->exec, c->stream));
    return RFE_OK;
}
std::string host_graph_key(const rfe_ctx* c, const char* kind, std::initializer_list<long long> v);

GemmArgs gemm_plain(const float* A, int lda, const float* Bw, int ldb, const float* bias, float* C, int ldc, int M, int N, int K);
GemmArgs gemm_lg(const float* A, int lda, const float* Bw, int ldb, const float* bias, float* C, int ldc, int M, int N, int K);
GemmArgs gemm_lgw(const rfe_ctx* c, const float* A, int lda, const float* Bw, int ldb, const float* bias, float* C, int ldc, int M, int N, int K);

struct SpBuffers {
    float *p1, *a2, *p2, *a3, *p3, *a4, *f4, *pa, *logits, *da, *dmap, *smap, *nmap, *ss;
    uint8_t *mask, *supp;
    float* cand_score; int32_t* cand_idx;
    unsigned long long* sel_keys; int32_t* sel_n;
    bool tail_fused = false;
};
size_t sp_ws_bytes(int B, int H, int W);
int sp_carve(rfe_ctx* c, int B, int H, int W, SpBuffers& b);
int sp_check(rfe_ctx* c, int H, int W, int B, int Kmax);
int sp_forward_maps(rfe_ctx* c, const void* img, int H, int W, int stride, int B, SpBuffers& b, bool join, bool& forked, bool img_f32 = false,
                    long long frame_step = 0 , float thr = 0.0005f ,
                    bool want_maps = false );
int sp_forward(rfe_ctx* c, const void* img, int H, int W, int stride, int B, int Kmax, float thr,
               int32_t* n, int32_t* kxy, float* score, float* desc, uint8_t* desc_bin = nullptr, bool img_f32 = false, long long frame_step = 0);

struct PyrPlan {
    int L = 0, Ktot = 0;
    int32_t h[RFE_MAX_LEVELS], w[RFE_MAX_LEVELS]; float s[RFE_MAX_LEVELS];
    int kmax[RFE_MAX_LEVELS]; bool run[RFE_MAX_LEVELS];
    size_t off[RFE_MAX_LEVELS];
    size_t frame = 0;
};
int pyr_check(rfe_ctx* c, int H, int W, int stride, int B, int L, float sf, const int32_t* kmax, PyrPlan& P);
int pyr_prepare(rfe_ctx* c, int H, int W, int B, float sf, const PyrPlan& P, bool own_levels);
int pyr_forward(rfe_ctx* c, const uint8_t* img, int H, int W, int stride, int B, const PyrPlan& P, float thr, uint8_t* lv, bool copy_level0,
                int32_t* n, int32_t* level_n, float* kpts, int32_t* octave, float* score, float* desc, long long img_frame = 0);

struct LgBuffers {
    float *x, *kn, *csn, *lnstat, *qkv, *ctx, *msg, *h, *md, *z, *sim, *rowlse, *collse, *mx0, *apart;
    int32_t *a0, *a1, *lens, *kvmap;
};
void lg_layout(Bump& a, int P, int L, LgBuffers& b);
inline size_t lg_ws_bytes(int P, int L) { LgBuffers b; return layout_bytes([&](Bump& a) { lg_layout(a, P, L, b); }); }
template <typename X> int lg_carve(rfe_ctx* c, int P, int L, LgBuffers& b, X&& extra) {
    return ws_carve(c, &c->ws_lg, &c->ws_lg_bytes, [&](Bump& a) { lg_layout(a, P, L, b); extra(a); });
}
inline int lg_carve(rfe_ctx* c, int P, int L, LgBuffers& b) { return lg_carve(c, P, L, b, [](Bump&) {}); }
int lg_check(rfe_ctx* c, int P, int Mmax, int Nmax);
void lg_ffn(rfe_ctx* c, LgBuffers& b, float* x, const float* second, int rows, const float* w1, const float* b1, const float* g,
            const float* be, const float* w2, const float* b2);
bool lg_self_qkv_attention(rfe_ctx* c, LgBuffers& b, const LgLayerDev& Lw, const float* x, const float* csn, const int32_t* lens, int nseq, int L);
void lg_self_block(rfe_ctx* c, LgBuffers& b, const LgLayerDev& Lw, float* x, const float* csn, const int32_t* lens, int nseq, int L);
int lg_forward(rfe_ctx* c, LgBuffers& b, int P, int L, float thr, int cap, int32_t* S, int32_t* pairs, float* ms,
               float* scores_opt, bool first_self_done = false, bool posenc_done = false);
void lg_assign_stage(hipStream_t s, LgBuffers& b, int P, int L, float thr, int cap, int32_t* S, int32_t* pairs, float* ms,
                     float* scores_opt, int scores_pair , const float* wm, const float* bm);
int lg_stage(rfe_ctx* c, LgBuffers& b, const float* k0n, const float* k1n, const float* d0, const float* d1,
             const int32_t* m, const int32_t* n, int P, int Mmax, int Nmax, int L);

}
```

rover-slam_amd/csrc/api_weights.hip:

```cpp
#include <stdio.h>
#include <stdlib.h>
#include <string.h>
#include <map>
#include <mutex>
#include <tuple>
#include "api_internal.h"

using namespace rfe;

extern "C" int64_t rfe_weight_count(int kind) {
    return kind == RFE_KIND_SUPERPOINT ? SP_COUNT : kind == RFE_KIND_LIGHTGLUE ? LG_COUNT : -1;
}

namespace {
struct SpShared {
    rfe::SpWeightsDev w; int device = 0; std::vector<float> host;
    ~SpShared() {
        (void)hipSetDevice(device);
        if (w.conv1a_w) (void)hipFree(w.conv1a_w);
        for (int l = 0; l < 12; ++l) { if (w.packed[l]) (void)hipFree(w.packed[l]); if (w.bias[l]) (void)hipFree(w.bias[l]); }
    }
};
struct LgShared {
    rfe::LgWeightsDev w; int device = 0; std::vector<float> host;
    ~LgShared() { (void)hipSetDevice(device); if (w.blob) (void)hipFree(w.blob); if (w.extra) (void)hipFree(w.extra); if (w.h2) (void)hipFree(w.h2); }
};
std::mutex g_weights_mu;
std::map<std::tuple<int, int, uint64_t, int>, std::weak_ptr<void>> g_weights;

uint64_t fnv1a64(const float* p, size_t n) {
    const unsigned char* b = reinterpret_cast<const unsigned char*>(p);
    uint64_t h = 1469598103934665603ull;
    for (size_t i = 0; i < n * sizeof(float); ++i) { h ^= b[i]; h *= 1099511628211ull; }
    return h;
}
}

static int upload(rfe_ctx* c, float** dst, const float* src, size_t n) {
    if (*dst) { RFE_HIP(c, hipFree(*dst)); *dst = nullptr; }
    RFE_HIP(c, hipMalloc((void**)dst, n * sizeof(float)));
    RFE_HIP(c, hipMemcpy(*dst, src, n * sizeof(float), hipMemcpyHostToDevice));
    return RFE_OK;
}

static int set_sp_upload(rfe_ctx* c, const float* blob);
static int set_lg_upload(rfe_ctx* c, const float* blob);

template <typename Shared, typename Dev>
static int set_shared(rfe_ctx* c, int kind, const float* blob, size_t count, std::shared_ptr<void>& hold, Dev& dev, bool& has, int (*upload_fn)(rfe_ctx*, const float*)) {
    const uint64_t hash = fnv1a64(blob, count);
    std::lock_guard<std::mutex> lk(g_weights_mu);
    auto key = std::make_tuple(c->device, kind, hash, 0);
    for (;; ++std::get<3>(key)) {
        auto it = g_weights.find(key);
        if (it == g_weights.end()) break;
        auto sp = it->second.lock();
        if (!sp) break;
        if (memcmp(static_cast<Shared*>(sp.get())->host.data(), blob, count * sizeof(float)) != 0) continue;
        hold = sp; dev = static_cast<Shared*>(sp.get())->w; has = true;
        return RFE_OK;
    }
    has = false; hold.reset(); dev = Dev();
    int rc = upload_fn(c, blob);
    auto sp = std::make_shared<Shared>();
    sp->w = dev; sp->device = c->device;
    if (rc) { dev = Dev(); return rc; }
    sp->host.assign(blob, blob + count);
    hold = sp; g_weights[key] = sp;
    return RFE_OK;
}
static int set_sp(rfe_ctx* c, const float* blob) {
    return set_shared<SpShared>(c, RFE_KIND_SUPERPOINT, blob, (size_t)SP_COUNT, c->sp_hold, c->sp, c->has_sp, set_sp_upload);
}
static int set_lg(rfe_ctx* c, const float* blob) {
    return set_shared<LgShared>(c, RFE_KIND_LIGHTGLUE, blob, (size_t)LG_COUNT, c->lg_hold, c->lg, c->has_lg, set_lg_upload);
}

static int set_sp_upload(rfe_ctx* c, const float* blob) {
    size_t off = 0;
    for (int l = 0; l < 12; ++l) {
        const SpLayer& L = kSpLayers[l];
        const float* w = blob + off;
        const size_t wn = (size_t)L.cout * L.cin * L.k * L.k;
        const float* b = w + wn;
        off += wn + L.cout;
        int rc;
        if (l == L_1A) {
            std::vector<float> t(9 * 64);
            for (int co = 0; co < 64; ++co) for (int k = 0; k < 9; ++k) t[k * 64 + co] = w[co * 9 + k];
            if ((rc = upload(c, &c->sp.conv1a_w, t.data(), t.size()))) return rc;
        } else if (L.k == 3) {
            std::vector<float> t;
            pack_conv3x3_weights(w, L.cin, L.cout, L.pool, t);
            if ((rc = upload(c, &c->sp.packed[l], t.data(), t.size()))) return rc;
        } else {
            if ((rc = upload(c, &c->sp.packed[l], w, wn))) return rc;
        }
        if ((rc = upload(c, &c->sp.bias[l], b, L.cout))) return rc;
    }
    c->has_sp = true;
    return RFE_OK;
}

static int set_lg_upload(rfe_ctx* c, const float* blob) {
    int rc = upload(c, &c->lg.blob, blob, (size_t)LG_COUNT);
    if (rc) return rc;
    size_t taken = 0;
    auto take = [&](size_t n) { float* r = c->lg.blob + taken; taken += n; return r; };
    LgWeightsDev& W = c->lg;
    W.wr = take(64);
    for (int l = 0; l < LG_LAYERS; ++l) {
        LgLayerDev& L = W.L[l];
        L.wqkv = take(768 * 256); L.bqkv = take(768); L.wo = take(256 * 256); L.bo = take(256);
        L.w1 = take(512 * 512); L.b1 = take(512); L.lng = take(512); L.lnb = take(512);
        L.w2 = take(256 * 512); L.b2 = take(256);
        L.cwqk = take(256 * 256); L.cbqk = take(256); L.cwv = take(256 * 256); L.cbv = take(256);
        L.cwo = take(256 * 256); L.cbo = take(256);
        L.cw1 = take(512 * 512); L.cb1 = take(512); L.clng = take(512); L.clnb = take(512);
        L.cw2 = take(256 * 512); L.cb2 = take(256);
    }
    W.wp = take(256 * 256); W.bp = take(256); W.wm = take(256); W.bm = take(1);
    if (taken != (size_t)LG_COUNT) return fail(c, RFE_ERR_INVALID, "internal: LightGlue blob layout mismatch");
    if (W.extra) { RFE_HIP(c, hipFree(W.extra)); W.extra = nullptr; }
    const size_t per = 512 * 256 + 512 + 2 * (512 * 512 + 512);
    RFE_HIP(c, hipMalloc((void**)&W.extra, per * LG_LAYERS * sizeof(float)));
    {
        std::vector<float> w1f(512 * 512), b1f(512);
        std::vector<double> acc(256);
        size_t off = 64;
        for (int l = 0; l < LG_LAYERS; ++l) {
            LgLayerDev& L = W.L[l];
            float* base = W.extra + per * l + 512 * 256 + 512;
            L.w1f = base; L.b1f = base + 512 * 512; L.cw1f = L.b1f + 512; L.cb1f = L.cw1f + 512 * 512;
            const float* h = blob + off;
            const float* s_wo = h + 768 * 256 + 768; const float* s_bo = s_wo + 256 * 256;
            const float* s_w1 = s_bo + 256; const float* s_b1 = s_w1 + 512 * 512;
            const float* cr = s_b1 + 512 + 512 + 512 + 256 * 512 + 256;
            const float* c_wo = cr + 2 * (256 * 256 + 256); const float* c_bo = c_wo + 256 * 256;
            const float* c_w1 = c_bo + 256; const float* c_b1 = c_w1 + 512 * 512;
            off += 1250560;
            for (int blk = 0; blk < 2; ++blk) {
                const float* wo = blk ? c_wo : s_wo; const float* bo = blk ? c_bo : s_bo;
                const float* w1 = blk ? c_w1 : s_w1; const float* b1 = blk ? c_b1 : s_b1;
                for (int i = 0; i < 512; ++i) {
                    const float* w1row = w1 + (size_t)i * 512;
                    for (int j = 0; j < 256; ++j) { w1f[(size_t)i * 512 + j] = w1row[j]; acc[j] = 0.0; }
                    double bacc = b1[i];
                    for (int k = 0; k < 256; ++k) {
                        const double wv = w1row[256 + k];
                        const float* worow = wo + (size_t)k * 256;
                        for (int j = 0; j < 256; ++j) acc[j] += wv * (double)worow[j];
                        bacc += wv * (double)bo[k];
                    }
                    for (int j = 0; j < 256; ++j) w1f[(size_t)i * 512 + 256 + j] = (float)acc[j];
                    b1f[i] = (float)bacc;
                }
                RFE_HIP(c, hipMemcpy(blk ? L.cw1f : L.w1f, w1f.data(), w1f.size() * 4, hipMemcpyHostToDevice));
                RFE_HIP(c, hipMemcpy(blk ? L.cb1f : L.b1f, b1f.data(), b1f.size() * 4, hipMemcpyHostToDevice));
            }
        }
    }
    for (int l = 0; l < LG_LAYERS; ++l) {
        LgLayerDev& L = W.L[l];
        L.cwqkv = W.extra + per * l; L.cbqkv = L.cwqkv + 512 * 256;
        RFE_HIP(c, hipMemcpy(L.cwqkv, L.cwqk, 256 * 256 * 4, hipMemcpyDeviceToDevice));
        RFE_HIP(c, hipMemcpy(L.cwqkv + 256 * 256, L.cwv, 256 * 256 * 4, hipMemcpyDeviceToDevice));
        RFE_HIP(c, hipMemcpy(L.cbqkv, L.cbqk, 256 * 4, hipMemcpyDeviceToDevice));
        RFE_HIP(c, hipMemcpy(L.cbqkv + 256, L.cbv, 256 * 4, hipMemcpyDeviceToDevice));
    }
    if (W.h2) { RFE_HIP(c, hipFree(W.h2)); W.h2 = nullptr; }
    W.n_blob = ((size_t)LG_COUNT + 63) & ~(size_t)63; W.n_extra = per * LG_LAYERS;
    RFE_HIP(c, hipMalloc((void**)&W.h2, 2 * (W.n_blob + W.n_extra) * sizeof(uint16_t)));
    launch_split_f16(c->stream, W.blob, W.h2, W.h2 + W.n_blob, (size_t)LG_COUNT);
    launch_split_f16(c->stream, W.extra, W.h2 + 2 * W.n_blob, W.h2 + 2 * W.n_blob + W.n_extra, W.n_extra);
    RFE_HIP(c, hipGetLastError());
    RFE_HIP(c, hipStreamSynchronize(c->stream));
    c->has_lg = true;
    return RFE_OK;
}

static void take_hparams(rfe_hparams& to, const rfe_hparams& from, int kind) {
    if (kind == RFE_KIND_SUPERPOINT) {
        to.sp_max_keypoints = from.sp_max_keypoints; to.sp_detection_threshold = from.sp_detection_threshold; to.sp_nms_radius = from.sp_nms_radius;
        to.sp_remove_borders = from.sp_remove_borders; to.sp_topk_always = from.sp_topk_always;
    } else {
        to.lg_layers = from.lg_layers; to.lg_heads = from.lg_heads; to.lg_filter_threshold = from.lg_filter_threshold;
    }
}

extern "C" int rfe_set_weights(rfe_ctx* c, int kind, const float* blob, int64_t count) {
    if (!c || !blob) return fail(c, RFE_ERR_INVALID, "rfe_set_weights: null argument");
    RFE_HIP(c, hipSetDevice(c->device));
    if (count != rfe_weight_count(kind)) return fail(c, RFE_ERR_INVALID, "rfe_set_weights: wrong float count for this model kind");
    RFE_HIP(c, hipStreamSynchronize(c->stream));
    const int rc = kind == RFE_KIND_SUPERPOINT ? set_sp(c, blob) : set_lg(c, blob);
    ++c->settings_gen;
    if (rc == RFE_OK) {
        take_hparams(c->hp, rfe_default_hparams(), kind);
    }
    return rc;
}

extern "C" uint64_t rfe_weights_id(rfe_ctx* c, int kind) {
    if (!c) return 0;
    const void* p = kind == RFE_KIND_SUPERPOINT ? c->sp_hold.get() : kind == RFE_KIND_LIGHTGLUE ? c->lg_hold.get() : nullptr;
    return (uint64_t)(uintptr_t)p;
}

static int check_hparams(rfe_ctx* c, const rfe_hparams& h, const char* who) {
    if (h.sp_max_keypoints < 1 || h.sp_max_keypoints > 4096) return fail(c, RFE_ERR_INVALID, std::string(who) + ": sp_max_keypoints must be in 1..4096");
    if (!(h.sp_detection_threshold >= 0.f) || !(h.sp_detection_threshold < 1.f)) return fail(c, RFE_ERR_INVALID, std::string(who) + ": sp_detection_threshold must be in [0, 1)");
    if (h.sp_nms_radius < 1 || h.sp_nms_radius > NMS_MAX_RADIUS) return fail(c, RFE_ERR_INVALID, std::string(who) + ": sp_nms_radius must be in 1.." + std::to_string(NMS_MAX_RADIUS));
    if (h.sp_remove_borders < 0 || h.sp_remove_borders > 64) return fail(c, RFE_ERR_INVALID, std::string(who) + ": sp_remove_borders must be in 0..64");
    if (h.sp_topk_always != 0 && h.sp_topk_always != 1) return fail(c, RFE_ERR_INVALID, std::string(who) + ": sp_topk_always must be 0 or 1");
    if (h.lg_layers != LG_LAYERS || h.lg_heads != 4)
        return fail(c, RFE_ERR_INVALID, std::string(who) + ": the LightGlue kernels are built for 9 layers of 4 heads x 64, the file / caller says " +
                                        std::to_string(h.lg_layers) + " layers of " + std::to_string(h.lg_heads) + " heads");
    if (!(h.lg_filter_threshold >= 0.f) || !(h.lg_filter_threshold < 1.f)) return fail(c, RFE_ERR_INVALID, std::string(who) + ": lg_filter_threshold must be in [0, 1)");
    return RFE_OK;
}

static int load_rfew(rfe_ctx* c, const char* path, int want_kind) {
    FILE* f = fopen(path, "rb");
    if (!f) return fail(c, RFE_ERR_IO, std::string("cannot open weight file ") + path);
    unsigned char head[20];
    if (fread(head, 1, 20, f) != 20 || memcmp(head, "RFEW", 4) != 0) { fclose(f); return fail(c, RFE_ERR_IO, std::string("not an RFEW file: ") + path); }
    uint32_t ver, kind; uint64_t cnt;
    memcpy(&ver, head + 4, 4); memcpy(&kind, head + 8, 4); memcpy(&cnt, head + 12, 8);
    if ((ver != 1 && ver != 2) || (int)kind != want_kind || (int64_t)cnt != rfe_weight_count(want_kind)) { fclose(f); return fail(c, RFE_ERR_IO, std::string("RFEW header mismatch in ") + path); }
    rfe_hparams hp = c->hp;
    if (ver == 2) {
        uint32_t hb = 0;
        unsigned char blk[256];
        const uint32_t need = want_kind == RFE_KIND_SUPERPOINT ? 20u : 12u;
        if (fread(&hb, 4, 1, f) != 1 || hb < need || hb > sizeof(blk) || fread(blk, 1, hb, f) != hb) { fclose(f); return fail(c, RFE_ERR_IO, std::string("RFEW v2 hyper-parameter block damaged in ") + path); }
        if (want_kind == RFE_KIND_SUPERPOINT) {
            memcpy(&hp.sp_max_keypoints, blk, 4); memcpy(&hp.sp_detection_threshold, blk + 4, 4);
            memcpy(&hp.sp_nms_radius, blk + 8, 4); memcpy(&hp.sp_remove_borders, blk + 12, 4); memcpy(&hp.sp_topk_always, blk + 16, 4);
        } else {
            memcpy(&hp.lg_layers, blk, 4); memcpy(&hp.lg_heads, blk + 4, 4); memcpy(&hp.lg_filter_threshold, blk + 8, 4);
        }
        const int rc = check_hparams(c, hp, path);
        if (rc) { fclose(f); c->err = "RFEW v2 hyper-parameters refused: " + c->err; return RFE_ERR_IO; }
    }
    std::vector<float> blob(cnt);
    size_t got = fread(blob.data(), sizeof(float), cnt, f);
    fclose(f);
    if (got != cnt) return fail(c, RFE_ERR_IO, std::string("short read on ") + path);
    const int rc = rfe_set_weights(c, want_kind, blob.data(), (int64_t)cnt);
    if (rc == RFE_OK && ver == 2) take_hparams(c->hp, hp, want_kind);
    return rc;
}

extern "C" int rfe_get_hparams(rfe_ctx* c, rfe_hparams* out) {
    if (!c || !out) return RFE_ERR_INVALID;
    *out = c->hp;
    return RFE_OK;
}
extern "C" int rfe_set_hparams(rfe_ctx* c, const rfe_hparams* in) {
    if (!c || !in) return RFE_ERR_INVALID;
    const int rc = check_hparams(c, *in, "rfe_set_hparams");
    if (rc) return rc;
    c->hp = *in;
    ++c->settings_gen;
    return RFE_OK;
}

static int load_onnx(rfe_ctx* c, const char* path, int want_kind) {
    std::vector<float> blob;
    rfe_hparams hp = rfe_default_hparams();
    std::string err;
    if (!rfe::onnx_convert(path, want_kind, blob, &hp, err)) return fail(c, RFE_ERR_IO, err);
    int rc = check_hparams(c, hp, path);
    if (rc) { c->err = "graph hyper-parameters refused: " + c->err; return RFE_ERR_IO; }
    if ((int64_t)blob.size() != rfe_weight_count(want_kind)) return fail(c, RFE_ERR_IO, std::string("converted weight count mismatch for ") + path);
    rc = rfe_set_weights(c, want_kind, blob.data(), (int64_t)blob.size());
    if (rc == RFE_OK) take_hparams(c->hp, hp, want_kind);
    return rc;
}

static int load_any(rfe_ctx* c, const char* path, int want_kind) {
    FILE* f = fopen(path, "rb");
    if (!f) return fail(c, RFE_ERR_IO, std::string("cannot open weight file ") + path);
    unsigned char magic[4] = {0, 0, 0, 0};
    const size_t got = fread(magic, 1, 4, f);
    fclose(f);
    if (got == 4 && memcmp(magic, "RFEW", 4) == 0) return load_rfew(c, path, want_kind);
    return load_onnx(c, path, want_kind);
}

static int load_pair(rfe_ctx* c, const char* sp_path, const char* lg_path, int (*load)(rfe_ctx*, const char*, int)) {
    if (!c) return RFE_ERR_INVALID;
    int rc;
    if (sp_path && (rc = load(c, sp_path, RFE_KIND_SUPERPOINT))) return rc;
    if (lg_path && (rc = load(c, lg_path, RFE_KIND_LIGHTGLUE))) return rc;
    return RFE_OK;
}
extern "C" int rfe_load_weights(rfe_ctx* c, const char* sp_path, const char* lg_path) { return load_pair(c, sp_path, lg_path, load_any); }
extern "C" int rfe_load_onnx(rfe_ctx* c, const char* sp_path, const char* lg_path) { return load_pair(c, sp_path, lg_path, load_onnx); }
```

rover-slam_amd/csrc/rfe_internal.h:

```cpp
#pragma once
#include <hip/hip_runtime.h>
#include <stdint.h>
#include <stdlib.h>
#include <memory>
#include <string>
#include <vector>
#include "../../include/rover_fe.h"

typedef float f32x16 __attribute__((ext_vector_type(16)));
typedef float f32x4 __attribute__((ext_vector_type(4)));

namespace rfe {


struct SpLayer { int cin, cout, k; bool pool; };
static const SpLayer kSpLayers[12] = {
    {1, 64, 3, false}, {64, 64, 3, true}, {64, 64, 3, false}, {64, 64, 3, true}, {64, 128, 3, false}, {128, 128, 3, true},
    {128, 128, 3, false}, {128, 128, 3, false}, {128, 256, 3, false}, {256, 65, 1, false}, {128, 256, 3, false}, {256, 256, 1, false}};
enum { L_1A, L_1B, L_2A, L_2B, L_3A, L_3B, L_4A, L_4B, L_PA, L_PB, L_DA, L_DB };

constexpr int LG_LAYERS = 9;
constexpr int64_t SP_COUNT = 1300865;
constexpr int64_t LG_COUNT = 11321153;

constexpr int CONV_CK = 8;
constexpr int CONV_NT = 64;

struct SpWeightsDev {
    float* conv1a_w = nullptr;
    float* packed[12] = {nullptr};
    float* bias[12] = {nullptr};
};

struct LgLayerDev {
    float *wqkv, *bqkv, *wo, *bo, *w1, *b1, *lng, *lnb, *w2, *b2;
    float *cwqk, *cbqk, *cwv, *cbv, *cwo, *cbo, *cw1, *cb1, *clng, *clnb, *cw2, *cb2;
    float *cwqkv, *cbqkv;
    float *w1f, *b1f, *cw1f, *cb1f;
};
struct LgWeightsDev {
    float* blob = nullptr;
    float* extra = nullptr;
    float* wr;
    LgLayerDev L[LG_LAYERS];
    float *wp, *bp, *wm, *bm;
    uint16_t* h2 = nullptr;
    size_t n_blob = 0, n_extra = 0;
};

struct Stage { std::string name; double ms = 0; int64_t calls = 0; };

struct GemmArgs {
    const float* A; int lda;
    const float* A2; int lda2; int K1;
    const float* B; int ldb;
    const float* bias;
    const float* R; int ldr;
    float* C; int ldc;
    int M, N, K;
    float alpha; int relu;
    long long sA, sA2, sB, sC, sR;
    const int* m_valid;
    int batch;
    float* stats_out;
    const float* stats_in; int stats_p; const float* ln_g; const float* ln_b;
    const uint16_t* Bh; const uint16_t* Bl;
    int kperm;
    const float* rope_csn; int rope_c0, rope_c1;
};

}

inline rfe_hparams rfe_default_hparams() { return rfe_hparams{1024, 0.0005f, 4, 4, 0, rfe::LG_LAYERS, 4, 0.1f}; }

struct rfe_ctx {
    int device = 0;
    hipStream_t own_stream = nullptr;
    hipStream_t stream = nullptr;
    hipStream_t side_stream = nullptr;
    hipEvent_t ev_fork = nullptr, ev_join = nullptr;
    hipEvent_t ev_pyr = nullptr;
    std::string err;
    bool has_sp = false, has_lg = false;
    bool opt_lg_fold = true;
    bool opt_lg_fp16x2 = false;
    bool opt_host_graph = false;
    struct HostGraph {
        struct Slot { std::string key; hipGraphExec_t exec = nullptr; unsigned long long used = 0; };
        struct Seen { std::string key; int count = 0; unsigned long long used = 0; };
        Slot slot[4]; Seen seen[8]; unsigned long long tick = 0;
    };
    HostGraph g_extract, g_match;
    unsigned long long settings_gen = 0;
    rfe_hparams hp = rfe_default_hparams();
    rfe::SpWeightsDev sp;
    rfe::LgWeightsDev lg;
    std::shared_ptr<void> sp_hold, lg_hold;
    void* ws_sp = nullptr; size_t ws_sp_bytes = 0;
    void* ws_lg = nullptr; size_t ws_lg_bytes = 0;
    void* ws_io = nullptr; size_t ws_io_bytes = 0;
    void* h_pin = nullptr; size_t h_pin_bytes = 0;
    void* ws_tmp = nullptr; size_t ws_tmp_bytes = 0;
    void* ws_pyr = nullptr; size_t ws_pyr_bytes = 0;
    void* ws_ptab = nullptr; size_t ws_ptab_bytes = 0; std::string ptab_key; std::vector<size_t> ptab_off;
    int32_t* sp_cnt = nullptr;
    bool sp_cnt_dirty = false;
    void* ws_ps = nullptr; size_t ws_ps_bytes = 0;
    int ps_cap = 0;
    void* ws_st = nullptr; size_t ws_st_bytes = 0;
    int st_H = 0, st_W = 0, st_K = 0; bool st_have_prev = false; int st_flip = 0; std::string st_pyr_key;
    struct { bool armed = false; int pair = 0; float *x0 = nullptr, *x1 = nullptr, *scores = nullptr; } tap;
    bool prof = false;
    std::string prof_filter;
    std::vector<rfe::Stage> stages;
    std::vector<std::pair<int, std::pair<hipEvent_t, hipEvent_t>>> pending;
    std::vector<hipEvent_t> ev_pool;
};

namespace rfe {

int fail(rfe_ctx* c, int code, const std::string& msg);
#define RFE_HIP(ctx, call)                                                                      \
    do {                                                                                        \
        hipError_t e_ = (call);                                                                 \
        if (e_ != hipSuccess)                                                                   \
            return rfe::fail((ctx), RFE_ERR_HIP, std::string(#call) + ": " + hipGetErrorString(e_)); \
    } while (0)

struct ProfScope {
    rfe_ctx* c; int idx; hipEvent_t e0 = nullptr, e1 = nullptr;
    hipStream_t st;
    ProfScope(rfe_ctx* ctx, const char* name, hipStream_t on = nullptr);
    ~ProfScope();
};
void prof_collect(rfe_ctx* c);

int ensure_ws(rfe_ctx* c, void** p, size_t* cur, size_t need);

bool conv3x3_reads_t16(int cin, int cout, bool pool);
void pack_conv3x3_weights(const float* w_oihw, int cin, int cout, bool pool, std::vector<float>& out);
size_t packed_conv3x3_count(int cin, int cout, bool pool);
void launch_conv3x3(hipStream_t s, const float* in, int B, int H, int W, int cin,
                    const float* wpacked, const float* bias, int cout, bool relu, bool pool, float* out,
                    int tag = 0);
void launch_conv1ab_fused(hipStream_t s, const void* img, bool img_f32, int stride, int B, int H, int W, const float* w1a,
                          const float* b1a, const float* wp, const float* bias, float* out, long long frame_step = 0 );
inline void ensure_dynamic_lds(const void* kernel, int bytes, bool* done) {
    int dev = 0;
    (void)hipGetDevice(&dev);
    if (dev < 0 || dev >= 64 || !done[dev]) {
        (void)hipFuncSetAttribute(kernel, hipFuncAttributeMaxDynamicSharedMemorySize, bytes);
        if (dev >= 0 && dev < 64) done[dev] = true;
    }
}
int launch_gemm_h2(hipStream_t s, const GemmArgs& g);
void launch_split_f16(hipStream_t s, const float* x, uint16_t* hi, uint16_t* lo, size_t n);
bool gemm_nt_rope_ok(const GemmArgs& g);
int launch_gemm_nt(hipStream_t s, const GemmArgs& g);
inline bool gemm_latency_regime(const GemmArgs& g) {
    const long long b = g.batch > 0 ? g.batch : 1;
    auto tiles = [&](int bm, int bn) { return (long long)((g.M + bm - 1) / bm) * ((g.N + bn - 1) / bn) * b; };
    const bool big = (g.N % 256 == 0 && tiles(128, 256) >= 256) || tiles(128, 128) >= 256 || g.M > 8192;
    return !big;
}
bool launch_gemm_lat(hipStream_t s, const GemmArgs& g, const float* rope_csn, int rope_cols);
bool onnx_convert(const std::string& path, int kind, std::vector<float>& blob, rfe_hparams* hp, std::string& err);
bool launch_ffn2_ln_lat(hipStream_t s, const float* h, const float* w2, const float* b2, const float* ln_g, const float* ln_b, const float* R, int ldr,
                        float* C, int ldc, int M);
bool launch_lg_attention_lat(hipStream_t s, const float* q, const float* k, const float* v, int ld, float* out, int nseq, int Lq, int Lk,
                             const int* qlen, const int* klen, const int* kv_map, bool h2 = false );
void launch_softmax65_d2s(hipStream_t s, const float* logits, int ld, int B, int Hc, int Wc, float* score);
constexpr int NMS_MAX_RADIUS = 8;
void launch_nms(hipStream_t s, const float* score, int B, int H, int W, int radius , int border, float* tmp_ss,
                uint8_t* tmp_mask, uint8_t* tmp_supp, float* out);
void launch_select(hipStream_t s, const float* nms, int B, int H, int W, int Kmax, float thr,
                   float* cand_score, int32_t* cand_idx, int32_t* n_out, int32_t* kxy, float* score,
                   int32_t* chunk_cnt , bool topk_always ,
                   unsigned long long* sel_keys , int32_t* sel_n );
bool launch_sp_tail_lat(hipStream_t s, const float* logits, int B, int Hc, int Wc, int radius, int border, float thr, unsigned long long* cand_keys ,
                        int32_t* cand_cnt , float* smap_out , float* nmap_out );
void launch_select_keys(hipStream_t s, const unsigned long long* cand_keys, int32_t* cand_cnt, int B, int H, int W, int Kmax, bool topk_always,
                        int32_t* n_out, int32_t* kxy, float* score);
void launch_keys_from_map(hipStream_t s, const float* nms, int B, int HW, float thr, unsigned long long* cand_keys, int32_t* cand_cnt);
void launch_descmap_norm(hipStream_t s, float* dmap, int64_t cells);
void launch_desc_sample(hipStream_t s, const float* dmap, int B, int Hc, int Wc, int H, int W,
                        const int32_t* n, const int32_t* kxy, int Kmax, float* desc, uint8_t* desc_bin );
void launch_lg_posenc(hipStream_t s, const float* kn, const float* wr, int rows, float* csn );
void launch_lg_attention(hipStream_t s, const float* q, const float* k, const float* v, int ld ,
                         float* out, int nseq, int Lq, int Lk, const int* qlen, const int* klen,
                         const int* kv_map ,
                         float* part ,
                         const float* rope_csn = nullptr ,
                         bool fp16x2 = false );
void launch_lg_attention_h2(hipStream_t s, const float* q, const float* k, const float* v, int ld, float* out, int nseq, int Lq, int Lk,
                            const int* qlen, const int* klen, const int* kv_map, const float* rope_csn);
size_t lg_attention_part_bytes(int nseq, int Lq);
void launch_lg_ln_gelu(hipStream_t s, float* h, const float* g, const float* b, int64_t rows);
void launch_lg_assign(hipStream_t s, const float* sim, const float* z0, const float* z1, int P, int L,
                      int cap, const int* m, const int* n, float thr, float* scores_opt, float* rowlse,
                      float* collse, int32_t* a0, float* mx0, int32_t* a1, int32_t* S, int32_t* pairs,
                      float* ms, int scores_pair ,
                      const float* x, const float* wm, const float* bm, float* z );
bool lg_assign_few_pairs(int P, int L);
void launch_lg_frame_prologue(hipStream_t s, const int32_t* kxy, const float* desc, const float* wr, const int32_t* nkp, int B, int L, int rows, int cols,
                              float* kn, float* csn, float* x, int32_t* lens, int32_t* kvmap);
void launch_lg_matchability(hipStream_t s, const float* x, const float* w, const float* b, int64_t rows, float* z);
void launch_copy_f32(hipStream_t s, const float* src, float* dst, int64_t n);
void launch_normalize_kpts(hipStream_t s, const int32_t* kxy, int64_t n, int rows, int cols, float* out);

void launch_stereo_match(hipStream_t s, const uint8_t* imgL, const uint8_t* imgR, int H, int W, int stride,
                         const float* kL, int N, const float* kR, int Nr, const float* dL, const float* dR, float mb,
                         float mbf, float* uRight, float* depth, int32_t* sadv);

void launch_stereo_match_counts(hipStream_t s, const uint8_t* imgL, const uint8_t* imgR, int H, int W, int stride,
                                const int32_t* kL, const int32_t* kR, int Kmax, const int32_t* counts, const float* dL,
                                const float* dR, float mb, float mbf, float* uRight, float* depth, int32_t* sadv);

int pyramid_geometry(int H, int W, int nlevels, float scale_factor, int32_t* level_h, int32_t* level_w, float* level_scale);
void pyramid_tables(int nlevels, const int32_t* level_h, const int32_t* level_w, std::vector<int2>& tab, std::vector<size_t>& off);
void launch_pyr_resample(hipStream_t s, const uint8_t* src, long long src_frame, int src_stride, int Hs, int Ws, uint8_t* dst, long long dst_frame,
                         int Hd, int Wd, int B, const int2* cx, const int2* cy);
struct PyrMergeArgs {
    int L, Ktot;
    const int32_t* n[RFE_MAX_LEVELS];
    const int32_t* kxy[RFE_MAX_LEVELS];
    const float* sc[RFE_MAX_LEVELS];
    const float* desc_l[RFE_MAX_LEVELS];
    int kmax[RFE_MAX_LEVELS];
    float scale[RFE_MAX_LEVELS];
    int32_t* n_out; int32_t* level_n ; float* kpts; int32_t* octave; float* score; float* desc;
};
void launch_pyr_merge(hipStream_t s, const PyrMergeArgs& a, int B);

struct StereoPyrTable {
    int L;
    int32_t h[RFE_MAX_LEVELS], w[RFE_MAX_LEVELS];
    uint32_t off[RFE_MAX_LEVELS];
    float s[RFE_MAX_LEVELS], inv[RFE_MAX_LEVELS];
};
void launch_stereo_match_pyr(hipStream_t s, const uint8_t* levL, const uint8_t* levR, const StereoPyrTable& T, const float* kL,
                             const int32_t* octL, int N, const float* kR, const int32_t* octR, int Nr, const int32_t* counts,
                             const float* dL, const float* dR, float mb, float mbf, int sad_level0, float* uRight, float* depth,
                             int32_t* sadv);

void launch_l2_matrix(hipStream_t s, const float* a, int M, const float* b, int N, float* out);
void launch_binarize(hipStream_t s, const float* d, int64_t rows, uint8_t* out);
void launch_search_candidates(hipStream_t s, const float* q, int Nq, const float* f, int Nf, const int32_t* offsets, const int32_t* cand,
                              const uint8_t* skip, int32_t* best_idx, float* best_dist, float* second_dist);
void launch_distinctive(hipStream_t s, const float* desc, const int32_t* offsets, int total , int Np, int maxn,
                        float* med , int32_t* best, float* median);

__device__ __forceinline__ float desc_dist_wave(const float4 a, const float4 b) {
    const float d0 = a.x - b.x, d1 = a.y - b.y, d2 = a.z - b.z, d3 = a.w - b.w;
    double p = 0.0;
    p += (double)d0 * (double)d0; p += (double)d1 * (double)d1; p += (double)d2 * (double)d2; p += (double)d3 * (double)d3;
#pragma unroll
    for (int off = 32; off >= 1; off >>= 1) p = p + __shfl_xor(p, off);
    return (float)sqrt(p);
}

void launch_proj_grid(hipStream_t s, const float* kpts, const int32_t* kxy, int Nf, const int32_t* nf_dev, float min_x, float min_y,
                      float inv_w, float inv_h, int32_t* cell_start, int32_t* cell_items, float* fxy);
void launch_proj_count(hipStream_t s, const float* proj, const float* radius, const int32_t* pred_level, int Nq, const int32_t* cell_start,
                       const int32_t* cell_items, const float* fxy, const int32_t* octave, float min_x, float min_y, float inv_w,
                       float inv_h, int cand_cap, int32_t* seg_off, int32_t* cand_idx, int32_t* stats);
void launch_proj_fill(hipStream_t s, const float* q, int Nq, const float* f, int Nf, const int32_t* seg_off, const int32_t* cand_idx,
                      const uint8_t* skip, float* cand_dist);
void launch_proj_fill_trunc(hipStream_t s, const float* q, int Nq, const float* f, int Nf, const int32_t* seg_off, const int32_t* cand_idx,
                            const uint8_t* skip, float* cand_dist);
void launch_proj_resolve(hipStream_t s, const int32_t* seg_off, const int32_t* cand_idx, const float* cand_dist, const uint8_t* observed,
                         int Nq, int Nf, float th_high, int32_t* assign, int32_t* best_idx, float* best_dist, float* second_dist,
                         int32_t* stats);

void launch_sim3_project(hipStream_t s, const rfe_sim3_params& P, const float* pw, const float* normal, const float* min_dist,
                         const float* max_dist, const float* scale_dist, const uint8_t* valid, int Np, float* proj, float* radius,
                         int32_t* level, int32_t* reject, int32_t* stats);

}
```

rover-slam_amd/csrc/sp_post.hip:

```cpp
#include "rfe_internal.h"
#include "dev_prims.h"

namespace rfe {

__device__ __forceinline__ float rfe_expf(float x) {
    x = fmaxf(x, -87.0f);
    x = fminf(x, 88.0f);
    const float n = rintf(x * 1.44269504088896341f);
    float r = fmaf(n, -0.693359375f, x);
    r = fmaf(n, 2.12194440e-4f, r);
    float p = 1.9875691500E-4f;
    p = fmaf(p, r, 1.3981999507E-3f);
    p = fmaf(p, r, 8.3334519073E-3f);
    p = fmaf(p, r, 4.1665795894E-2f);
    p = fmaf(p, r, 1.6666665459E-1f);
    p = fmaf(p, r, 5.0000001201E-1f);
    const float r2 = r * r;
    const float y = fmaf(p, r2, r) + 1.0f;
    return y * __uint_as_float((uint32_t)((int)n + 127) << 23);
}

__global__ __launch_bounds__(256) void softmax65_d2s_kernel(const float* __restrict__ logits, int ld,
                                                            int cells_total, int Hc, int Wc,
                                                            float* __restrict__ score) {
// ... 526 lines not shown

void launch_select(hipStream_t s, const float* nms, int B, int H, int W, int Kmax, float thr, float* cand_score,
                   int32_t* cand_idx, int32_t* n_out, int32_t* kxy, float* score, int32_t* chunk_cnt, bool topk_always,
                   unsigned long long* sel_keys, int32_t* sel_n) {
    int P2 = 1;
    while (P2 < Kmax) P2 <<= 1;
    const int HW = H * W, nch = (HW + SEL_CHUNK - 1) / SEL_CHUNK;
    hipLaunchKernelGGL(select_count_kernel, dim3(nch, B), dim3(256), 0, s, nms, HW, nch, thr, chunk_cnt);
    hipLaunchKernelGGL(select_compact_kernel, dim3(nch, B), dim3(256), 0, s, nms, HW, nch, thr, chunk_cnt, cand_score, cand_idx);
    constexpr int SELECT_RANKALL_FRAMES = 4;
    if (B <= SELECT_RANKALL_FRAMES) {
        const int cap = HW < RA_MAX ? HW : RA_MAX, span = cap > Kmax ? cap : Kmax;
        static bool ls_[64];
        ensure_dynamic_lds((const void*)select_rankall_kernel, RA_MAX * 8, ls_);
        hipLaunchKernelGGL(select_rankall_kernel, dim3((span + RA_PER - 1) / RA_PER, B), dim3(256), (size_t)cap * 8, s, cand_score, cand_idx, chunk_cnt, nch, HW, W,
                           Kmax, topk_always ? 1 : 0, n_out, kxy, score);
        return;
    }
    hipLaunchKernelGGL(select_kernel, dim3(B), dim3(SEL_T), (size_t)P2 * 8, s, nms, H, W, Kmax, P2, thr,
                       cand_score, cand_idx, n_out, kxy, score, chunk_cnt, nch, topk_always ? 1 : 0, sel_keys, sel_n);
    hipLaunchKernelGGL(select_rank_kernel, dim3((Kmax + 63) / 64, B), dim3(256), (size_t)Kmax * 8, s, sel_keys, sel_n, W, Kmax, kxy, score);
}


constexpr int ST_NT = 1024;
template <int TH_>
__global__ __launch_bounds__(ST_NT, 1) void sp_tail_lat_kernel(const float* __restrict__ logits, int Hc, int Wc, int border, float thr,
                                                               unsigned long long* __restrict__ cand_keys, int32_t* __restrict__ cand_cnt,
                                                               float* __restrict__ smap_out, float* __restrict__ nmap_out) {
    constexpr int NF_IH = TH_ + 2 * NF_HALO;
    constexpr int NCY = (NF_IH + 7) / 8 + 1, NCX = (NF_IW + 7) / 8 + 1;
    static_assert(NF_IH % 4 == 0, "quad items");
    static_assert(NCY * NCX * 65 <= 3 * NF_IH * NF_IW, "the exponentials live in the T | Mk | SS planes");
    static_assert(ST_NT == SEL_T, "block scan");
    extern __shared__ __attribute__((aligned(16))) float nf_lds[];
    float* const S = nf_lds;
    float* const T = S + NF_IH * NF_IW;
    float* const Mk = T + NF_IH * NF_IW;
    float* const SS = Mk + NF_IH * NF_IW;
    uint8_t* const SUP = reinterpret_cast<uint8_t*>(SS + NF_IH * NF_IW);
    float* const E = T;
    __shared__ float cmax[NCY * NCX], csum[NCY * NCX];
    __shared__ int wtot[ST_NT / 64];
    __shared__ int sbase;
    const int H = 8 * Hc, W = 8 * Wc, HW = H * W;
    const int b = blockIdx.z;
    const size_t fo = (size_t)b * HW;
    const int y0 = blockIdx.y * TH_ - NF_HALO, x0 = blockIdx.x * NTW - NF_HALO;
    const int tid = threadIdx.x;
    const int cy_lo = y0 > 0 ? y0 >> 3 : 0, cx_lo = x0 > 0 ? x0 >> 3 : 0;
    int cy_hi = (y0 + NF_IH - 1) >> 3; cy_hi = cy_hi < Hc - 1 ? cy_hi : Hc - 1;
    int cx_hi = (x0 + NF_IW - 1) >> 3; cx_hi = cx_hi < Wc - 1 ? cx_hi : Wc - 1;
    const int ncy = cy_hi - cy_lo + 1, ncx = cx_hi - cx_lo + 1, ncell = ncy * ncx, rowlen = ncx * 65;
    {
        const float* lb = logits + ((size_t)b * Hc * Wc) * 65;
        for (int r = 0; r < ncy; ++r) {
            const float* src = lb + ((size_t)(cy_lo + r) * Wc + cx_lo) * 65;
            for (int j = tid; j < rowlen; j += ST_NT) E[r * rowlen + j] = src[j];
        }
    }
    __syncthreads();
    for (int cell = tid; cell < ncell; cell += ST_NT) {
        const float* e = E + cell * 65;
        float m = e[0];
#pragma unroll
        for (int c = 0; c < 65; ++c) m = fmaxf(m, e[c]);
        cmax[cell] = m;
    }
    __syncthreads();
    for (int i = tid; i < ncell * 65; i += ST_NT) E[i] = rfe_expf(E[i] - cmax[i / 65]);
    __syncthreads();
    for (int cell = tid; cell < ncell; cell += ST_NT) {
        const float* e = E + cell * 65;
        float sm = 0.f;
#pragma unroll
        for (int c = 0; c < 65; ++c) sm = sm + e[c];
        csum[cell] = sm;
    }
    __syncthreads();
    for (int idx = tid; idx < NF_IH * NF_IW; idx += ST_NT) {
        const int py = idx / NF_IW, px = idx % NF_IW, gy = y0 + py, gx = x0 + px;
        float v = -INFINITY;
        if (gy >= 0 && gy < H && gx >= 0 && gx < W) {
            const int cell = ((gy >> 3) - cy_lo) * ncx + ((gx >> 3) - cx_lo);
            v = E[cell * 65 + (gy & 7) * 8 + (gx & 7)] / csum[cell];
            if (smap_out && py >= NF_HALO && py < NF_HALO + TH_ && px >= NF_HALO && px < NF_HALO + NTW) smap_out[fo + (size_t)gy * W + gx] = v;
        }
        S[idx] = v;
    }
    __syncthreads();
    auto inside = [&](int py, int px) { const int gy = y0 + py, gx = x0 + px; return gy >= 0 && gy < H && gx >= 0 && gx < W; };
    nf_rowpass<0, NF_IH, ST_NT>(S, T, tid);
    __syncthreads();
    nf_colpass<NF_R, NF_IH, ST_NT>(T, tid, [&](int py, int px, float m) {
        const int o = py * NF_IW + px;
        Mk[o] = inside(py, px) ? (S[o] == m ? 1.f : 0.f) : -INFINITY;
    });
    __syncthreads();
    nf_rowpass<NF_R, NF_IH, ST_NT>(Mk, T, tid);
    __syncthreads();
    nf_colpass<2 * NF_R, NF_IH, ST_NT>(T, tid, [&](int py, int px, float m) {
        const int o = py * NF_IW + px;
        const bool sp = m > 0.f;
        SUP[o] = sp ? 1 : 0;
        SS[o] = inside(py, px) ? (sp ? 0.f : S[o]) : -INFINITY;
    });
    __syncthreads();
    nf_rowpass<2 * NF_R, NF_IH, ST_NT>(SS, T, tid);
    __syncthreads();
    nf_colpass<3 * NF_R, NF_IH, ST_NT>(T, tid, [&](int py, int px, float m) {
        const int o = py * NF_IW + px;
        if (inside(py, px)) Mk[o] = (Mk[o] != 0.f || (SS[o] == m && !SUP[o])) ? 1.f : 0.f;
    });
    __syncthreads();
    nf_rowpass<3 * NF_R, NF_IH, ST_NT>(Mk, T, tid);
    __syncthreads();
    nf_colpass<4 * NF_R, NF_IH, ST_NT>(T, tid, [&](int py, int px, float m) {
        const int o = py * NF_IW + px;
        const bool sp = m > 0.f;
        SUP[o] = sp ? 1 : 0;
        SS[o] = inside(py, px) ? (sp ? 0.f : S[o]) : -INFINITY;
    });
    __syncthreads();
    nf_rowpass<4 * NF_R, NF_IH, ST_NT>(SS, T, tid);
    __syncthreads();
    nf_colpass<5 * NF_R, NF_IH, ST_NT>(T, tid, [&](int py, int px, float m) {
        const int o = py * NF_IW + px;
        if (!inside(py, px)) return;
        const bool mk = Mk[o] != 0.f || (SS[o] == m && !SUP[o]);
        const int gy = y0 + py, gx = x0 + px;
        float v = mk ? S[o] : 0.f;
        if (gy < border || gy >= H - border || gx < border || gx >= W - border) v = -1.f;
        Mk[o] = v;
        if (nmap_out) nmap_out[fo + (size_t)gy * W + gx] = v;
    });
    __syncthreads();
    constexpr int PPT = (TH_ * NTW + ST_NT - 1) / ST_NT;
    float cv[PPT]; int ci[PPT];
    int cnt = 0;
#pragma unroll
    for (int k = 0; k < PPT; ++k) {
        const int p = tid + k * ST_NT;
        cv[k] = -INFINITY; ci[k] = 0;
        if (p < TH_ * NTW) {
            const int py = NF_HALO + p / NTW, px = NF_HALO + p % NTW;
            const float v = Mk[py * NF_IW + px];
            cv[k] = v; ci[k] = (y0 + py) * W + (x0 + px);
        }
        cnt += cv[k] > thr ? 1 : 0;
    }
    int total;
    int pos = block_excl_scan_int(cnt, wtot, total);
    if (tid == 0) sbase = total > 0 ? atomicAdd(cand_cnt + 2 * b, total) : 0;
    __syncthreads();
    pos += sbase;
    unsigned long long* ck = cand_keys + fo;
#pragma unroll
    for (int k = 0; k < PPT; ++k)
        if (cv[k] > thr) { ck[pos] = ((unsigned long long)__float_as_uint(cv[k]) << 32) | (unsigned long long)(0xFFFFFFFFu - (unsigned int)ci[k]); ++pos; }
}

__global__ __launch_bounds__(256) void select_rankall_keys_kernel(const unsigned long long* __restrict__ cand_keys, int32_t* __restrict__ cand_cnt,
                                                                  int HW, int W, int Kmax, int topk_always, int32_t* __restrict__ n_out,
                                                                  int32_t* __restrict__ kxy, float* __restrict__ score) {
    extern __shared__ __attribute__((aligned(16))) unsigned char smem[];
    unsigned long long* keys = reinterpret_cast<unsigned long long*>(smem);
    const int b = blockIdx.y, tid = threadIdx.x;
    const int count = cand_cnt[2 * b];
    const unsigned long long* ck = cand_keys + (size_t)b * HW;
    int32_t* okxy = kxy + (size_t)b * Kmax * 2;
    float* osc = score + (size_t)b * Kmax;
    const int nsel = count < Kmax ? count : Kmax;
    if (blockIdx.x == 0 && tid == 0) n_out[b] = nsel;
    const int span = count > Kmax ? count : Kmax;
    const int nwin = (count + RA_MAX - 1) / RA_MAX;
    const bool rowmajor = count <= Kmax && !topk_always;
    auto xf = [&](unsigned long long k) { return rowmajor ? (k << 32) | (k >> 32) : k; };
    auto load_window = [&](int w0, int wn) {
        const u64x2* src = reinterpret_cast<const u64x2*>(ck + w0);
        u64x2* dst = reinterpret_cast<u64x2*>(keys);
        const int npair = wn >> 1;
        for (int j0 = tid; j0 < npair; j0 += 8 * 256) {
            u64x2 t[8];
#pragma unroll
            for (int u = 0; u < 8; ++u) { const int j = j0 + u * 256; t[u] = j < npair ? src[j] : u64x2{0ull, 0ull}; }
#pragma unroll
            for (int u = 0; u < 8; ++u) { const int j = j0 + u * 256; if (j < npair) dst[j] = u64x2{xf(t[u][0]), xf(t[u][1])}; }
        }
        if ((wn & 1) && tid == 0) keys[wn - 1] = xf(ck[w0 + wn - 1]);
    };
    bool loaded = false;
    for (int t0 = blockIdx.x * RA_PER; t0 < span; t0 += gridDim.x * RA_PER) {
        const int t = t0 + (tid >> 3), part = tid & 7;
        if (part == 0 && t >= nsel && t < Kmax) { okxy[2 * t] = 0; okxy[2 * t + 1] = 0; osc[t] = 0.f; }
        if (t0 >= count) continue;
        const bool live = t < count;
        const unsigned long long key = live ? xf(ck[t]) : ~0ull;
        const u64x2* kp = reinterpret_cast<const u64x2*>(keys);
        int rank = 0;
        for (int w = 0; w < nwin; ++w) {
            const int w0 = w * RA_MAX, wn = count - w0 < RA_MAX ? count - w0 : RA_MAX;
            if (nwin > 1 || !loaded) {
                if (loaded) __syncthreads();
                load_window(w0, wn);
                loaded = true;
                __syncthreads();
            }
            const int npair = wn >> 1;
#pragma unroll 8
            for (int j = part; j < npair; j += 8) { const u64x2 kk = kp[j]; rank += (kk[0] > key ? 1 : 0) + (kk[1] > key ? 1 : 0); }
            if ((wn & 1) && part == 0) rank += keys[wn - 1] > key ? 1 : 0;
        }
        rank += __shfl_xor(rank, 1);
        rank += __shfl_xor(rank, 2);
        rank += __shfl_xor(rank, 4);
        if (live && part == 0 && rank < Kmax) {
            const unsigned long long k0 = rowmajor ? (key << 32) | (key >> 32) : key;
            const int idx = (int)(0xFFFFFFFFu - (unsigned int)(k0 & 0xFFFFFFFFull));
            okxy[2 * rank] = idx % W; okxy[2 * rank + 1] = idx / W;
            osc[rank] = __uint_as_float((unsigned int)(k0 >> 32));
        }
    }
    __syncthreads();
    if (tid == 0) {
        __threadfence();
        const int tk = atomicAdd(cand_cnt + 2 * b + 1, 1);
        if (tk == (int)gridDim.x - 1) { cand_cnt[2 * b] = 0; cand_cnt[2 * b + 1] = 0; __threadfence(); }
    }
}

bool launch_sp_tail_lat(hipStream_t st, const float* logits, int B, int Hc, int Wc, int radius, int border, float thr, unsigned long long* cand_keys,
                        int32_t* cand_cnt, float* smap_out, float* nmap_out) {
    constexpr int SP_TAIL_FUSED_FRAMES = 4;
    if (radius != NF_R || B > SP_TAIL_FUSED_FRAMES || B < 1) return false;
    const int H = 8 * Hc, W = 8 * Wc;
    const int gx = (W + NTW - 1) / NTW;
    auto wgs = [&](int th) { return (long long)gx * ((H + th - 1) / th) * B; };
    const int th = wgs(32) <= 256 ? 32 : wgs(40) <= 256 ? 40 : wgs(48) <= 256 ? 48 : 32;
#define RFE_SP_TAIL_GO(TH_)                                                                                                                  \
    do {                                                                                                                                     \
        constexpr int bytes = (TH_ + 2 * NF_HALO) * NF_IW * 17;                                                                               \
        static bool ls_[64];                                                                                                                 \
        ensure_dynamic_lds((const void*)sp_tail_lat_kernel<TH_>, bytes, ls_);                                                                \
        hipLaunchKernelGGL(sp_tail_lat_kernel<TH_>, dim3(gx, (H + TH_ - 1) / TH_, B), dim3(ST_NT), bytes, st, logits, Hc, Wc, border, thr,   \
                           cand_keys, cand_cnt, smap_out, nmap_out);                                                                         \
    } while (0)
    if (th == 48) RFE_SP_TAIL_GO(48);
    else if (th == 40) RFE_SP_TAIL_GO(40);
    else RFE_SP_TAIL_GO(32);
#undef RFE_SP_TAIL_GO
    return true;
}

__global__ __launch_bounds__(256) void keys_from_map_kernel(const float* __restrict__ nms, int HW, float thr, unsigned long long* __restrict__ cand_keys,
                                                            int32_t* __restrict__ cand_cnt) {
    const int b = blockIdx.y;
    const long long t = (long long)blockIdx.x * 256 + threadIdx.x;
    if (t >= HW) return;
    const int p = (int)((t * 7919 + 13) % HW);
    const float v = nms[(size_t)b * HW + p];
    if (v > thr) {
        const int pos = atomicAdd(cand_cnt + 2 * b, 1);
        cand_keys[(size_t)b * HW + pos] = ((unsigned long long)__float_as_uint(v) << 32) | (unsigned long long)(0xFFFFFFFFu - (unsigned int)p);
    }
}
void launch_keys_from_map(hipStream_t s, const float* nms, int B, int HW, float thr, unsigned long long* cand_keys, int32_t* cand_cnt) {
    hipLaunchKernelGGL(keys_from_map_kernel, dim3((HW + 255) / 256, B), dim3(256), 0, s, nms, HW, thr, cand_keys, cand_cnt);
}

void launch_select_keys(hipStream_t s, const unsigned long long* cand_keys, int32_t* cand_cnt, int B, int H, int W, int Kmax, bool topk_always,
                        int32_t* n_out, int32_t* kxy, float* score) {
    const int HW = H * W;
    const int cap = HW < RA_MAX ? HW : RA_MAX, span = cap > Kmax ? cap : Kmax;
    static bool ls_[64];
    ensure_dynamic_lds((const void*)select_rankall_keys_kernel, RA_MAX * 8, ls_);
    hipLaunchKernelGGL(select_rankall_keys_kernel, dim3((span + RA_PER - 1) / RA_PER, B), dim3(256), (size_t)cap * 8, s, cand_keys, cand_cnt, HW, W, Kmax,
                       topk_always ? 1 : 0, n_out, kxy, score);
}

__device__ __forceinline__ float wave_sumsq256(float4 v) {
    float p = v.x * v.x;
    p = fmaf(v.y, v.y, p);
    p = fmaf(v.z, v.z, p);
    p = fmaf(v.w, v.w, p);
#pragma unroll
    for (int off = 32; off >= 1; off >>= 1) p = p + __shfl_xor(p, off);
    return p;
}

__global__ __launch_bounds__(256) void descmap_norm_kernel(float* __restrict__ dmap, int64_t cells) {
    const int64_t cell = (int64_t)blockIdx.x * 4 + (threadIdx.x >> 6);
    if (cell >= cells) return;
    const int lane = threadIdx.x & 63;
    float4* p = reinterpret_cast<float4*>(dmap + cell * 256) + lane;
    float4 v = *p;
    const float d = fmaxf(sqrtf(wave_sumsq256(v)), 1e-12f);
    v.x = v.x / d; v.y = v.y / d; v.z = v.z / d; v.w = v.w / d;
    *p = v;
}
void launch_descmap_norm(hipStream_t s, float* dmap, int64_t cells) {
    hipLaunchKernelGGL(descmap_norm_kernel, dim3((unsigned)((cells + 3) / 4)), dim3(256), 0, s, dmap, cells);
}

__global__ __launch_bounds__(256) void desc_sample_kernel(const float* __restrict__ dmap, int Hc, int Wc, int H, int W,
                                                          const int32_t* __restrict__ n, const int32_t* __restrict__ kxy,
                                                          int Kmax, float* __restrict__ desc, uint8_t* __restrict__ desc_bin) {
    const int b = blockIdx.y;
    const int k = blockIdx.x * 4 + (threadIdx.x >> 6);
    if (k >= Kmax) return;
    const int lane = threadIdx.x & 63;
    float4* o = reinterpret_cast<float4*>(desc + ((size_t)b * Kmax + k) * 256) + lane;
    uchar4* ob = desc_bin ? reinterpret_cast<uchar4*>(desc_bin + ((size_t)b * Kmax + k) * 256) + lane : nullptr;
    if (k >= n[b]) { *o = make_float4(0.f, 0.f, 0.f, 0.f); if (ob) *ob = make_uchar4(0, 0, 0, 0); return; }
    const int x = kxy[((size_t)b * Kmax + k) * 2], y = kxy[((size_t)b * Kmax + k) * 2 + 1];
    const float gx = (((float)x - 3.5f) / ((float)W - 4.5f)) * 2.0f - 1.0f;
    const float gy = (((float)y - 3.5f) / ((float)H - 4.5f)) * 2.0f - 1.0f;
    const float ix = ((gx + 1.0f) * 0.5f) * (float)(Wc - 1);
    const float iy = ((gy + 1.0f) * 0.5f) * (float)(Hc - 1);
    const float fx0 = floorf(ix), fy0 = floorf(iy);
    const int x0 = (int)fx0, y0 = (int)fy0, x1 = x0 + 1, y1 = y0 + 1;
    const float wx1 = ix - fx0, wy1 = iy - fy0, wx0 = (fx0 + 1.0f) - ix, wy0 = (fy0 + 1.0f) - iy;
    const float wnw = wx0 * wy0, wne = wx1 * wy0, wsw = wx0 * wy1, wse = wx1 * wy1;
    const float4 z = make_float4(0.f, 0.f, 0.f, 0.f);
    const float* mb = dmap + (size_t)b * Hc * Wc * 256;
    const bool vx0 = x0 >= 0 && x0 < Wc, vx1 = x1 >= 0 && x1 < Wc, vy0 = y0 >= 0 && y0 < Hc, vy1 = y1 >= 0 && y1 < Hc;
    const float4 nw = (vx0 && vy0) ? reinterpret_cast<const float4*>(mb + ((size_t)y0 * Wc + x0) * 256)[lane] : z;
    const float4 ne = (vx1 && vy0) ? reinterpret_cast<const float4*>(mb + ((size_t)y0 * Wc + x1) * 256)[lane] : z;
    const float4 sw = (vx0 && vy1) ? reinterpret_cast<const float4*>(mb + ((size_t)y1 * Wc + x0) * 256)[lane] : z;
    const float4 se = (vx1 && vy1) ? reinterpret_cast<const float4*>(mb + ((size_t)y1 * Wc + x1) * 256)[lane] : z;
    float4 v;
    v.x = fmaf(se.x, wse, fmaf(sw.x, wsw, fmaf(ne.x, wne, nw.x * wnw)));
    v.y = fmaf(se.y, wse, fmaf(sw.y, wsw, fmaf(ne.y, wne, nw.y * wnw)));
    v.z = fmaf(se.z, wse, fmaf(sw.z, wsw, fmaf(ne.z, wne, nw.z * wnw)));
    v.w = fmaf(se.w, wse, fmaf(sw.w, wsw, fmaf(ne.w, wne, nw.w * wnw)));
    const float d = fmaxf(sqrtf(wave_sumsq256(v)), 1e-12f);
    v.x = v.x / d; v.y = v.y / d; v.z = v.z / d; v.w = v.w / d;
    *o = v;
    if (ob) *ob = make_uchar4(v.x > 0.f, v.y > 0.f, v.z > 0.f, v.w > 0.f);
}
void launch_desc_sample(hipStream_t s, const float* dmap, int B, int Hc, int Wc, int H, int W, const int32_t* n,
                        const int32_t* kxy, int Kmax, float* desc, uint8_t* desc_bin) {
    hipLaunchKernelGGL(desc_sample_kernel, dim3((Kmax + 3) / 4, B), dim3(256), 0, s, dmap, Hc, Wc, H, W, n, kxy, Kmax, desc, desc_bin);
}

}
```

Baseline: 947.8 frames/s.

## Compute SuperPoint descriptor head only at cells touched by keypoints

For batches larger than four, the dense descriptor head (3x3 conv plus 1x1 GEMM plus normalisation over every cell) is skipped. Instead it marks the cells that bilinear sampling of the selected keypoints touches, compacts them into rows, gathers im2col patches and runs the two descriptor GEMMs only on those rows. Sampling then looks up compacted rows through a cell-to-row map. This cuts descriptor-head FLOPs and the side-stream fork. In exchange it serialises the head after keypoint selection and adds several small kernels plus the patch gather.

```diff
diff --git a/include/rover_fe.h b/include/rover_fe.h
--- a/include/rover_fe.h
+++ b/include/rover_fe.h
@@ -218,6 +218,8 @@
 int rfe_k_scoremap(rfe_ctx* ctx, const uint8_t* img_dev, int H, int W, int stride, int B,
                    float* scoremap_dev ,
                    float* nms_dev , float* descmap_dev );
+int rfe_k_sparse_desc(rfe_ctx* ctx, const uint8_t* img_dev, int H, int W, int stride, int B, int Kmax, const int32_t* n_dev, const int32_t* kxy_dev,
+                      int poison, int32_t* cell_row_dev, int32_t* count_dev, float* rows_dev, float* desc_dev);
 int rfe_k_select(rfe_ctx* ctx, const float* nms_dev , int B, int H, int W, int Kmax, float thr, int topk_always,
                  int32_t* n_dev, int32_t* kxy_dev, float* score_dev);
 int rfe_k_select_keys(rfe_ctx* ctx, const float* nms_dev , int B, int H, int W, int Kmax, float thr, int topk_always,
diff --git a/rover-slam_amd/capi.py b/rover-slam_amd/capi.py
--- a/rover-slam_amd/capi.py
+++ b/rover-slam_amd/capi.py
@@ -24,7 +24,7 @@
     "rfe_pool_create", "rfe_pool_destroy", "rfe_pool_last_error", "rfe_pool_size", "rfe_pool_ctx", "rfe_pool_has_rccl", "rfe_pool_set_weights",
     "rfe_pool_load_weights", "rfe_pool_set_option", "rfe_pool_set_hparams", "rfe_pool_shard", "rfe_pool_extract_match_stream",
     "rfe_profile_enable", "rfe_profile_filter", "rfe_profile_reset", "rfe_profile_read",
-    "rfe_k_conv3x3", "rfe_k_linear", "rfe_k_scoremap", "rfe_k_select", "rfe_k_select_keys", "rfe_k_lightglue_taps", "rfe_k_set_lightglue_tap", "rfe_k_lightglue_ffn", "rfe_k_attention", "rfe_k_lightglue_self_attention", "rfe_k_lightglue_assign", "rfe_k_pool_inject_gather_failure", "rfe_k_onnx_convert",
+    "rfe_k_conv3x3", "rfe_k_linear", "rfe_k_scoremap", "rfe_k_sparse_desc", "rfe_k_select", "rfe_k_select_keys", "rfe_k_lightglue_taps", "rfe_k_set_lightglue_tap", "rfe_k_lightglue_ffn", "rfe_k_attention", "rfe_k_lightglue_self_attention", "rfe_k_lightglue_assign", "rfe_k_pool_inject_gather_failure", "rfe_k_onnx_convert",
 ]
 
 if not os.path.exists(LIB_PATH):
@@ -146,6 +146,7 @@
 lib.rfe_k_conv3x3.argtypes = [C.c_void_p, _fp, C.c_int, C.c_int, C.c_int, C.c_int, _fp, _fp, C.c_int, C.c_int, C.c_int, _fp]
 lib.rfe_k_linear.argtypes = [C.c_void_p, _fp, C.c_int, C.c_int, _fp, _fp, C.c_int, C.c_int, _fp]
 lib.rfe_k_scoremap.argtypes = [C.c_void_p, _u8p, C.c_int, C.c_int, C.c_int, C.c_int, _fp, _fp, _fp]
+lib.rfe_k_sparse_desc.argtypes = [C.c_void_p, _u8p, C.c_int, C.c_int, C.c_int, C.c_int, C.c_int, _ip, _ip, C.c_int, _ip, _ip, _fp, _fp]
 lib.rfe_k_select.argtypes = [C.c_void_p, _fp, C.c_int, C.c_int, C.c_int, C.c_int, C.c_float, C.c_int, _ip, _ip, _fp]
 lib.rfe_k_select_keys.argtypes = lib.rfe_k_select.argtypes
 lib.rfe_k_lightglue_taps.argtypes = [C.c_void_p, _fp, _fp, _fp, _fp, C.c_int, C.c_int, _fp, _fp, _fp]
diff --git a/rover-slam_amd/csrc/api_extract.hip b/rover-slam_amd/csrc/api_extract.hip
--- a/rover-slam_amd/csrc/api_extract.hip
+++ b/rover-slam_amd/csrc/api_extract.hip
@@ -16,6 +16,8 @@
     b.mask = a.take<uint8_t>(hw); b.supp = a.take<uint8_t>(hw);
     b.cand_score = a.take<float>(hw); b.cand_idx = a.take<int32_t>(hw);
     b.sel_keys = a.take<unsigned long long>((size_t)B * 4096); b.sel_n = a.take<int32_t>(B);
+    b.cell_row = a.take<int32_t>(cells); b.row_cell = a.take<int32_t>(cells); b.cell_cnt = a.take<int32_t>(2 * (size_t)B + 1);
+    b.patch = b.p1;
 }
 size_t sp_ws_bytes(int B, int H, int W) { SpBuffers b; return layout_bytes([&](Bump& a) { sp_layout(a, B, H, W, b); }); }
 int sp_carve(rfe_ctx* c, int B, int H, int W, SpBuffers& b) {
@@ -39,7 +41,7 @@
 }
 
 int sp_forward_maps(rfe_ctx* c, const void* img, int H, int W, int stride, int B, SpBuffers& b, bool join, bool& forked, bool img_f32, long long frame_step,
-                    float thr, bool want_maps) {
+                    float thr, bool want_maps, bool dense_head) {
     forked = false;
     int rc = sp_carve(c, B, H, W, b);
     if (rc) return rc;
@@ -54,12 +56,14 @@
     { ProfScope p(c, "conv3b"); launch_conv3x3(s, b.a3, B, H2, W2, 128, w.packed[L_3B], w.bias[L_3B], 128, true, kSpLayers[L_3B].pool, b.p3, L_3B); }
     { ProfScope p(c, "conv4a"); launch_conv3x3(s, b.p3, B, Hc, Wc, 128, w.packed[L_4A], w.bias[L_4A], 128, true, kSpLayers[L_4A].pool, b.a4, L_4A); }
     { ProfScope p(c, "conv4b"); launch_conv3x3(s, b.a4, B, Hc, Wc, 128, w.packed[L_4B], w.bias[L_4B], 128, true, kSpLayers[L_4B].pool, b.f4, L_4B); }
-    const bool fork = !(c->prof && c->prof_filter.empty());
+    const bool fork = dense_head && !(c->prof && c->prof_filter.empty());
     hipStream_t sd = fork ? c->side_stream : s;
     if (fork) { RFE_HIP(c, hipEventRecord(c->ev_fork, s)); RFE_HIP(c, hipStreamWaitEvent(sd, c->ev_fork, 0)); }
-    { ProfScope p(c, "convDa", sd); launch_conv3x3(sd, b.f4, B, Hc, Wc, 128, w.packed[L_DA], w.bias[L_DA], 256, true, kSpLayers[L_DA].pool, b.da, L_DA); }
-    { ProfScope p(c, "convDb", sd); launch_gemm_nt(sd, gemm_plain(b.da, 256, w.packed[L_DB], 256, w.bias[L_DB], b.dmap, 256, cells, 256, 256)); }
-    { ProfScope p(c, "sp_post", sd); launch_descmap_norm(sd, b.dmap, cells); }
+    if (dense_head) {
+        { ProfScope p(c, "convDa", sd); launch_conv3x3(sd, b.f4, B, Hc, Wc, 128, w.packed[L_DA], w.bias[L_DA], 256, true, kSpLayers[L_DA].pool, b.da, L_DA); }
+        { ProfScope p(c, "convDb", sd); launch_gemm_nt(sd, gemm_plain(b.da, 256, w.packed[L_DB], 256, w.bias[L_DB], b.dmap, 256, cells, 256, 256)); }
+        { ProfScope p(c, "sp_post", sd); launch_descmap_norm(sd, b.dmap, cells); }
+    }
     if (fork) RFE_HIP(c, hipEventRecord(c->ev_join, sd));
     { ProfScope p(c, "convPa"); launch_conv3x3(s, b.f4, B, Hc, Wc, 128, w.packed[L_PA], w.bias[L_PA], 256, true, kSpLayers[L_PA].pool, b.pa, L_PA); }
     { ProfScope p(c, "convPb"); launch_gemm_nt(s, gemm_plain(b.pa, 256, w.packed[L_PB], 256, w.bias[L_PB], b.logits, 65, cells, 65, 256)); }
@@ -81,11 +85,33 @@
     return RFE_OK;
 }
 
+int sp_desc_rows(rfe_ctx* c, SpBuffers& b, int B, int Hc, int Wc, int Kmax, const int32_t* n, const int32_t* kxy) {
+    hipStream_t s = c->stream;
+    const SpWeightsDev& w = c->sp;
+    const int cap = sp_desc_cap(Kmax, Hc, Wc);
+    int32_t* const row_base = b.cell_cnt + B;
+    { ProfScope p(c, "sp_desc_cells");
+      launch_desc_cells(s, B, Hc, Wc, 8 * Hc, 8 * Wc, n, kxy, Kmax, cap, b.cell_row, b.row_cell, b.cell_cnt, row_base);
+      launch_desc_gather(s, b.f4, B, Hc, Wc, cap, b.row_cell, b.cell_cnt, row_base, b.patch); }
+    { ProfScope p(c, "convDa_rows");
+      GemmArgs g = gemm_plain(b.patch, 1152, w.da_rows, 1152, w.bias[L_DA], b.da, 256, B * cap, 256, 1152);
+      g.relu = 1; g.m_valid = row_base + B;
+      launch_gemm_nt(s, g); }
+    { ProfScope p(c, "convDb_rows");
+      GemmArgs g = gemm_plain(b.da, 256, w.packed[L_DB], 256, w.bias[L_DB], b.dmap, 256, B * cap, 256, 256);
+      g.m_valid = row_base + B;
+      launch_gemm_nt(s, g); }
+    { ProfScope p(c, "sp_desc_norm"); launch_descrows_norm(s, b.dmap, B, cap, b.cell_cnt, row_base); }
+    RFE_HIP(c, hipGetLastError());
+    return RFE_OK;
+}
+
 int sp_forward(rfe_ctx* c, const void* img, int H, int W, int stride, int B, int Kmax, float thr,
                int32_t* n, int32_t* kxy, float* score, float* desc, uint8_t* desc_bin, bool img_f32, long long frame_step) {
     SpBuffers b;
     bool forked;
-    int rc = sp_forward_maps(c, img, H, W, stride, B, b, false, forked, img_f32, frame_step, thr);
+    const bool sparse = B > 4;
+    int rc = sp_forward_maps(c, img, H, W, stride, B, b, false, forked, img_f32, frame_step, thr, false, !sparse);
     if (rc) return rc;
     const int Hc = H / 2 / 2 / 2, Wc = W / 2 / 2 / 2, Hs = 8 * Hc, Ws = 8 * Wc;
     { ProfScope p(c, "sp_select");
@@ -95,7 +121,12 @@
       } else
       launch_select(c->stream, b.nmap, B, Hs, Ws, Kmax, thr, b.cand_score, b.cand_idx, n, kxy, score, (int32_t*)b.ss , c->hp.sp_topk_always != 0, b.sel_keys, b.sel_n);
       if (forked) RFE_HIP(c, hipStreamWaitEvent(c->stream, c->ev_join, 0));
-      launch_desc_sample(c->stream, b.dmap, B, Hc, Wc, Hs, Ws, n, kxy, Kmax, desc, desc_bin); }
+      if (!sparse) launch_desc_sample(c->stream, b.dmap, B, Hc, Wc, Hs, Ws, n, kxy, Kmax, desc, desc_bin); }
+    if (sparse) {
+        if ((rc = sp_desc_rows(c, b, B, Hc, Wc, Kmax, n, kxy))) return rc;
+        ProfScope p(c, "sp_desc_sample");
+        launch_desc_sample(c->stream, b.dmap, B, Hc, Wc, Hs, Ws, n, kxy, Kmax, desc, desc_bin, b.cell_row, b.cell_cnt + B);
+    }
     RFE_HIP(c, hipGetLastError());
     return RFE_OK;
 }
diff --git a/rover-slam_amd/csrc/api_hooks.hip b/rover-slam_amd/csrc/api_hooks.hip
--- a/rover-slam_amd/csrc/api_hooks.hip
+++ b/rover-slam_amd/csrc/api_hooks.hip
@@ -52,6 +52,33 @@
     if (nms) RFE_HIP(c, hipMemcpyAsync(nms, b.nmap, hw * 4, hipMemcpyDeviceToDevice, c->stream));
     if (descmap) RFE_HIP(c, hipMemcpyAsync(descmap, b.dmap, hw / 64 * 256 * 4, hipMemcpyDeviceToDevice, c->stream));
     RFE_HIP(c, hipStreamSynchronize(c->stream));
+    return RFE_OK;
+}
+
+extern "C" int rfe_k_sparse_desc(rfe_ctx* c, const uint8_t* img, int H, int W, int stride, int B, int Kmax, const int32_t* n, const int32_t* kxy, int poison,
+                                 int32_t* cell_row, int32_t* count, float* rows, float* desc) {
+    int rc = sp_check(c, H, W, B, Kmax);
+    if (rc) return rc;
+    if (!img || !n || !kxy || stride < W) return fail(c, RFE_ERR_INVALID, "k_sparse_desc: null pointer or stride < W");
+    RFE_HIP(c, hipSetDevice(c->device));
+    SpBuffers b;
+    bool forked;
+    if ((rc = sp_forward_maps(c, img, H, W, stride, B, b, true, forked, false, 0, 0.0005f, false, false))) return rc;
+    const int Hc = H / 8, Wc = W / 8, cap = sp_desc_cap(Kmax, Hc, Wc);
+    const size_t cells = (size_t)B * Hc * Wc, live = (size_t)B * cap;
+    hipStream_t s = c->stream;
+    if (poison) {
+        const struct { void* p; size_t words; } fill[] = {{b.patch, live * 1152}, {b.da, cells * 256}, {b.dmap, cells * 256}, {b.cell_row, cells},
+                                                          {b.row_cell, cells}, {b.cell_cnt, (size_t)2 * B + 1}};
+        for (const auto& f : fill) RFE_HIP(c, hipMemsetD32Async((hipDeviceptr_t)f.p, -1, f.words, s));
+    }
+    if ((rc = sp_desc_rows(c, b, B, Hc, Wc, Kmax, n, kxy))) return rc;
+    if (desc) launch_desc_sample(s, b.dmap, B, Hc, Wc, 8 * Hc, 8 * Wc, n, kxy, Kmax, desc, nullptr, b.cell_row, b.cell_cnt + B);
+    RFE_HIP(c, hipGetLastError());
+    if (cell_row) RFE_HIP(c, hipMemcpyAsync(cell_row, b.cell_row, cells * 4, hipMemcpyDeviceToDevice, s));
+    if (count) RFE_HIP(c, hipMemcpyAsync(count, b.cell_cnt, (size_t)B * 4, hipMemcpyDeviceToDevice, s));
+    if (rows) RFE_HIP(c, hipMemcpyAsync(rows, b.dmap, live * 256 * 4, hipMemcpyDeviceToDevice, s));
+    RFE_HIP(c, hipStreamSynchronize(s));
     return RFE_OK;
 }
 
diff --git a/rover-slam_amd/csrc/api_internal.h b/rover-slam_amd/csrc/api_internal.h
--- a/rover-slam_amd/csrc/api_internal.h
+++ b/rover-slam_amd/csrc/api_internal.h
@@ -107,13 +107,17 @@
     float* cand_score; int32_t* cand_idx;
     unsigned long long* sel_keys; int32_t* sel_n;
     bool tail_fused = false;
+    int32_t *cell_row, *row_cell, *cell_cnt; float* patch;
 };
+inline int sp_desc_cap(int Kmax, int Hc, int Wc) { return std::min(4 * Kmax, Hc * Wc); }
 size_t sp_ws_bytes(int B, int H, int W);
 int sp_carve(rfe_ctx* c, int B, int H, int W, SpBuffers& b);
 int sp_check(rfe_ctx* c, int H, int W, int B, int Kmax);
 int sp_forward_maps(rfe_ctx* c, const void* img, int H, int W, int stride, int B, SpBuffers& b, bool join, bool& forked, bool img_f32 = false,
                     long long frame_step = 0 , float thr = 0.0005f ,
-                    bool want_maps = false );
+                    bool want_maps = false ,
+                    bool dense_head = true );
+int sp_desc_rows(rfe_ctx* c, SpBuffers& b, int B, int Hc, int Wc, int Kmax, const int32_t* n, const int32_t* kxy);
 int sp_forward(rfe_ctx* c, const void* img, int H, int W, int stride, int B, int Kmax, float thr,
                int32_t* n, int32_t* kxy, float* score, float* desc, uint8_t* desc_bin = nullptr, bool img_f32 = false, long long frame_step = 0);
 
diff --git a/rover-slam_amd/csrc/api_weights.hip b/rover-slam_amd/csrc/api_weights.hip
--- a/rover-slam_amd/csrc/api_weights.hip
+++ b/rover-slam_amd/csrc/api_weights.hip
@@ -18,6 +18,7 @@
     ~SpShared() {
         (void)hipSetDevice(device);
         if (w.conv1a_w) (void)hipFree(w.conv1a_w);
+        if (w.da_rows) (void)hipFree(w.da_rows);
         for (int l = 0; l < 12; ++l) { if (w.packed[l]) (void)hipFree(w.packed[l]); if (w.bias[l]) (void)hipFree(w.bias[l]); }
     }
 };
@@ -93,6 +94,7 @@
             std::vector<float> t;
             pack_conv3x3_weights(w, L.cin, L.cout, L.pool, t);
             if ((rc = upload(c, &c->sp.packed[l], t.data(), t.size()))) return rc;
+            if (l == L_DA && (rc = upload(c, &c->sp.da_rows, w, wn))) return rc;
         } else {
             if ((rc = upload(c, &c->sp.packed[l], w, wn))) return rc;
         }
diff --git a/rover-slam_amd/csrc/rfe_internal.h b/rover-slam_amd/csrc/rfe_internal.h
--- a/rover-slam_amd/csrc/rfe_internal.h
+++ b/rover-slam_amd/csrc/rfe_internal.h
@@ -30,6 +30,7 @@
     float* conv1a_w = nullptr;
     float* packed[12] = {nullptr};
     float* bias[12] = {nullptr};
+    float* da_rows = nullptr;
 };
 
 struct LgLayerDev {
@@ -184,7 +185,14 @@
 void launch_keys_from_map(hipStream_t s, const float* nms, int B, int HW, float thr, unsigned long long* cand_keys, int32_t* cand_cnt);
 void launch_descmap_norm(hipStream_t s, float* dmap, int64_t cells);
 void launch_desc_sample(hipStream_t s, const float* dmap, int B, int Hc, int Wc, int H, int W,
-                        const int32_t* n, const int32_t* kxy, int Kmax, float* desc, uint8_t* desc_bin );
+                        const int32_t* n, const int32_t* kxy, int Kmax, float* desc, uint8_t* desc_bin ,
+                        const int32_t* cell_row = nullptr ,
+                        const int32_t* row_base = nullptr );
+void launch_desc_cells(hipStream_t s, int B, int Hc, int Wc, int H, int W, const int32_t* n, const int32_t* kxy, int Kmax, int cap, int32_t* cell_row,
+                       int32_t* row_cell, int32_t* count, int32_t* row_base);
+void launch_desc_gather(hipStream_t s, const float* f4, int B, int Hc, int Wc, int cap, const int32_t* row_cell, const int32_t* count, const int32_t* row_base,
+                        float* patch);
+void launch_descrows_norm(hipStream_t s, float* rows, int B, int cap, const int32_t* count, const int32_t* row_base);
 void launch_lg_posenc(hipStream_t s, const float* kn, const float* wr, int rows, float* csn );
 void launch_lg_attention(hipStream_t s, const float* q, const float* k, const float* v, int ld ,
                          float* out, int nseq, int Lq, int Lk, const int* qlen, const int* klen,
diff --git a/rover-slam_amd/csrc/sp_post.hip b/rover-slam_amd/csrc/sp_post.hip
--- a/rover-slam_amd/csrc/sp_post.hip
+++ b/rover-slam_amd/csrc/sp_post.hip
@@ -852,9 +852,23 @@
     hipLaunchKernelGGL(descmap_norm_kernel, dim3((unsigned)((cells + 3) / 4)), dim3(256), 0, s, dmap, cells);
 }
 
+struct DescFoot { float ix, iy, fx0, fy0; int x0, y0, x1, y1; bool vx0, vx1, vy0, vy1; };
+__device__ __forceinline__ DescFoot desc_footprint(int x, int y, int H, int W, int Hc, int Wc) {
+    DescFoot f;
+    const float gx = (((float)x - 3.5f) / ((float)W - 4.5f)) * 2.0f - 1.0f;
+    const float gy = (((float)y - 3.5f) / ((float)H - 4.5f)) * 2.0f - 1.0f;
+    f.ix = ((gx + 1.0f) * 0.5f) * (float)(Wc - 1);
+    f.iy = ((gy + 1.0f) * 0.5f) * (float)(Hc - 1);
+    f.fx0 = floorf(f.ix); f.fy0 = floorf(f.iy);
+    f.x0 = (int)f.fx0; f.y0 = (int)f.fy0; f.x1 = f.x0 + 1; f.y1 = f.y0 + 1;
+    f.vx0 = f.x0 >= 0 && f.x0 < Wc; f.vx1 = f.x1 >= 0 && f.x1 < Wc; f.vy0 = f.y0 >= 0 && f.y0 < Hc; f.vy1 = f.y1 >= 0 && f.y1 < Hc;
+    return f;
+}
+
 __global__ __launch_bounds__(256) void desc_sample_kernel(const float* __restrict__ dmap, int Hc, int Wc, int H, int W,
                                                           const int32_t* __restrict__ n, const int32_t* __restrict__ kxy,
-                                                          int Kmax, float* __restrict__ desc, uint8_t* __restrict__ desc_bin) {
+                                                          int Kmax, float* __restrict__ desc, uint8_t* __restrict__ desc_bin,
+                                                          const int32_t* __restrict__ cell_row, const int32_t* __restrict__ row_base) {
     const int b = blockIdx.y;
     const int k = blockIdx.x * 4 + (threadIdx.x >> 6);
     if (k >= Kmax) return;
@@ -863,21 +877,23 @@
     uchar4* ob = desc_bin ? reinterpret_cast<uchar4*>(desc_bin + ((size_t)b * Kmax + k) * 256) + lane : nullptr;
     if (k >= n[b]) { *o = make_float4(0.f, 0.f, 0.f, 0.f); if (ob) *ob = make_uchar4(0, 0, 0, 0); return; }
     const int x = kxy[((size_t)b * Kmax + k) * 2], y = kxy[((size_t)b * Kmax + k) * 2 + 1];
-    const float gx = (((float)x - 3.5f) / ((float)W - 4.5f)) * 2.0f - 1.0f;
-    const float gy = (((float)y - 3.5f) / ((float)H - 4.5f)) * 2.0f - 1.0f;
-    const float ix = ((gx + 1.0f) * 0.5f) * (float)(Wc - 1);
-    const float iy = ((gy + 1.0f) * 0.5f) * (float)(Hc - 1);
-    const float fx0 = floorf(ix), fy0 = floorf(iy);
-    const int x0 = (int)fx0, y0 = (int)fy0, x1 = x0 + 1, y1 = y0 + 1;
+    const DescFoot f = desc_footprint(x, y, H, W, Hc, Wc);
+    const float ix = f.ix, iy = f.iy, fx0 = f.fx0, fy0 = f.fy0;
     const float wx1 = ix - fx0, wy1 = iy - fy0, wx0 = (fx0 + 1.0f) - ix, wy0 = (fy0 + 1.0f) - iy;
     const float wnw = wx0 * wy0, wne = wx1 * wy0, wsw = wx0 * wy1, wse = wx1 * wy1;
     const float4 z = make_float4(0.f, 0.f, 0.f, 0.f);
-    const float* mb = dmap + (size_t)b * Hc * Wc * 256;
-    const bool vx0 = x0 >= 0 && x0 < Wc, vx1 = x1 >= 0 && x1 < Wc, vy0 = y0 >= 0 && y0 < Hc, vy1 = y1 >= 0 && y1 < Hc;
-    const float4 nw = (vx0 && vy0) ? reinterpret_cast<const float4*>(mb + ((size_t)y0 * Wc + x0) * 256)[lane] : z;
-    const float4 ne = (vx1 && vy0) ? reinterpret_cast<const float4*>(mb + ((size_t)y0 * Wc + x1) * 256)[lane] : z;
-    const float4 sw = (vx0 && vy1) ? reinterpret_cast<const float4*>(mb + ((size_t)y1 * Wc + x0) * 256)[lane] : z;
-    const float4 se = (vx1 && vy1) ? reinterpret_cast<const float4*>(mb + ((size_t)y1 * Wc + x1) * 256)[lane] : z;
+    const float* mb = cell_row ? dmap + (size_t)row_base[b] * 256 : dmap + (size_t)b * Hc * Wc * 256;
+    const int32_t* cr = cell_row ? cell_row + (size_t)b * Hc * Wc : nullptr;
+    auto corner = [&](bool valid, int yy, int xx) {
+        if (!valid) return z;
+        int r = yy * Wc + xx;
+        if (cr) { r = cr[r]; if (r < 0) return z; }
+        return reinterpret_cast<const float4*>(mb + (size_t)r * 256)[lane];
+    };
+    const float4 nw = corner(f.vx0 && f.vy0, f.y0, f.x0);
+    const float4 ne = corner(f.vx1 && f.vy0, f.y0, f.x1);
+    const float4 sw = corner(f.vx0 && f.vy1, f.y1, f.x0);
+    const float4 se = corner(f.vx1 && f.vy1, f.y1, f.x1);
     float4 v;
     v.x = fmaf(se.x, wse, fmaf(sw.x, wsw, fmaf(ne.x, wne, nw.x * wnw)));
     v.y = fmaf(se.y, wse, fmaf(sw.y, wsw, fmaf(ne.y, wne, nw.y * wnw)));
@@ -889,8 +905,108 @@
     if (ob) *ob = make_uchar4(v.x > 0.f, v.y > 0.f, v.z > 0.f, v.w > 0.f);
 }
 void launch_desc_sample(hipStream_t s, const float* dmap, int B, int Hc, int Wc, int H, int W, const int32_t* n,
-                        const int32_t* kxy, int Kmax, float* desc, uint8_t* desc_bin) {
-    hipLaunchKernelGGL(desc_sample_kernel, dim3((Kmax + 3) / 4, B), dim3(256), 0, s, dmap, Hc, Wc, H, W, n, kxy, Kmax, desc, desc_bin);
-}
-
-}
+                        const int32_t* kxy, int Kmax, float* desc, uint8_t* desc_bin, const int32_t* cell_row, const int32_t* row_base) {
+    hipLaunchKernelGGL(desc_sample_kernel, dim3((Kmax + 3) / 4, B), dim3(256), 0, s, dmap, Hc, Wc, H, W, n, kxy, Kmax, desc, desc_bin, cell_row, row_base);
+}
+
+__global__ __launch_bounds__(256) void desc_cells_kernel(int Hc, int Wc, int H, int W, const int32_t* __restrict__ n, const int32_t* __restrict__ kxy, int Kmax,
+                                                         int cap, int32_t* __restrict__ cell_row, int32_t* __restrict__ row_cell, int32_t* __restrict__ count) {
+    __shared__ int wsum[4];
+    __shared__ int base_s;
+    const int b = blockIdx.x, tid = threadIdx.x, lane = tid & 63, wave = tid >> 6;
+    const int cells = Hc * Wc;
+    int32_t* cr = cell_row + (size_t)b * cells;
+    int32_t* rc = row_cell + (size_t)b * cap;
+    for (int c = tid; c < cells; c += 256) cr[c] = 0;
+    if (tid == 0) base_s = 0;
+    __syncthreads();
+    int nk = n[b]; nk = nk < Kmax ? nk : Kmax;
+    for (int k = tid; k < nk; k += 256) {
+        const DescFoot f = desc_footprint(kxy[((size_t)b * Kmax + k) * 2], kxy[((size_t)b * Kmax + k) * 2 + 1], H, W, Hc, Wc);
+        if (f.vx0 && f.vy0) cr[f.y0 * Wc + f.x0] = 1;
+        if (f.vx1 && f.vy0) cr[f.y0 * Wc + f.x1] = 1;
+        if (f.vx0 && f.vy1) cr[f.y1 * Wc + f.x0] = 1;
+        if (f.vx1 && f.vy1) cr[f.y1 * Wc + f.x1] = 1;
+    }
+    __syncthreads();
+    for (int c0 = 0; c0 < cells; c0 += 256) {
+        const int c = c0 + tid;
+        const bool m = c < cells && cr[c] != 0;
+        const unsigned long long bal = __ballot(m);
+        const int before = __popcll(bal & ((1ull << lane) - 1ull));
+        if (lane == 0) wsum[wave] = __popcll(bal);
+        __syncthreads();
+        int off = base_s;
+        for (int w = 0; w < wave; ++w) off += wsum[w];
+        const int total = wsum[0] + wsum[1] + wsum[2] + wsum[3];
+        if (c < cells) {
+            const int r = off + before;
+            const bool live = m && r < cap;
+            cr[c] = live ? r : -1;
+            if (live) rc[r] = c;
+        }
+        __syncthreads();
+        if (tid == 0) base_s += total;
+    }
+    __syncthreads();
+    if (tid == 0) count[b] = base_s < cap ? base_s : cap;
+}
+__global__ __launch_bounds__(64) void desc_row_base_kernel(const int32_t* __restrict__ count, int B, int32_t* __restrict__ row_base) {
+    const int lane = threadIdx.x;
+    int carry = 0;
+    for (int j0 = 0; j0 < B; j0 += 64) {
+        const int j = j0 + lane, v = j < B ? count[j] : 0;
+        int sum = v;
+#pragma unroll
+        for (int o = 1; o < 64; o <<= 1) { const int t = __shfl_up(sum, o); if (lane >= o) sum += t; }
+        if (j < B) row_base[j] = carry + sum - v;
+        carry += __shfl(sum, 63);
+    }
+    if (lane == 0) row_base[B] = carry;
+}
+void launch_desc_cells(hipStream_t s, int B, int Hc, int Wc, int H, int W, const int32_t* n, const int32_t* kxy, int Kmax, int cap, int32_t* cell_row,
+                       int32_t* row_cell, int32_t* count, int32_t* row_base) {
+    hipLaunchKernelGGL(desc_cells_kernel, dim3(B), dim3(256), 0, s, Hc, Wc, H, W, n, kxy, Kmax, cap, cell_row, row_cell, count);
+    hipLaunchKernelGGL(desc_row_base_kernel, dim3(1), dim3(64), 0, s, count, B, row_base);
+}
+
+__global__ __launch_bounds__(256) void desc_gather_kernel(const float* __restrict__ f4, int Hc, int Wc, int cap, const int32_t* __restrict__ row_cell,
+                                                          const int32_t* __restrict__ count, const int32_t* __restrict__ row_base, float* __restrict__ patch) {
+    const int b = blockIdx.y;
+    const int t = blockIdx.x * 256 + threadIdx.x;
+    const int r = t / 288, q = t - r * 288;
+    if (r >= count[b]) return;
+    const int cell = row_cell[(size_t)b * cap + r];
+    const int y = cell / Wc, x = cell - y * Wc;
+    const float* fb = f4 + (size_t)b * Hc * Wc * 128;
+    float v[4];
+#pragma unroll
+    for (int e = 0; e < 4; ++e) {
+        const int kappa = q * 4 + e, ci = kappa / 9, tap = kappa - ci * 9, ky = tap / 3, kx = tap - ky * 3;
+        const int yy = y + ky - 1, xx = x + kx - 1;
+        v[e] = (yy >= 0 && yy < Hc && xx >= 0 && xx < Wc) ? fb[((size_t)yy * Wc + xx) * 128 + ci] : 0.0f;
+    }
+    *reinterpret_cast<float4*>(patch + ((size_t)row_base[b] + r) * 1152 + q * 4) = make_float4(v[0], v[1], v[2], v[3]);
+}
+void launch_desc_gather(hipStream_t s, const float* f4, int B, int Hc, int Wc, int cap, const int32_t* row_cell, const int32_t* count, const int32_t* row_base,
+                        float* patch) {
+    hipLaunchKernelGGL(desc_gather_kernel, dim3((unsigned)(((long long)cap * 288 + 255) / 256), B), dim3(256), 0, s, f4, Hc, Wc, cap, row_cell, count, row_base,
+                       patch);
+}
+
+__global__ __launch_bounds__(256) void descrows_norm_kernel(float* __restrict__ rows, const int32_t* __restrict__ count, const int32_t* __restrict__ row_base) {
+    const int b = blockIdx.y;
+    const int r = blockIdx.x * 4 + (threadIdx.x >> 6);
+    if (r >= count[b]) return;
+    const int lane = threadIdx.x & 63;
+    float4* p = reinterpret_cast<float4*>(rows + ((size_t)row_base[b] + r) * 256) + lane;
+    float4 v = *p;
+    const float d = fmaxf(sqrtf(wave_sumsq256(v)), 1e-12f);
+    v.x = v.x / d; v.y = v.y / d; v.z = v.z / d; v.w = v.w / d;
+    *p = v;
+}
+void launch_descrows_norm(hipStream_t s, float* rows, int B, int cap, const int32_t* count, const int32_t* row_base) {
+    hipLaunchKernelGGL(descrows_norm_kernel, dim3((cap + 3) / 4, B), dim3(256), 0, s, rows, count, row_base);
+}
+
+}
```

After: 960.3 frames/s, median of 6. 1.3% higher.
